# qwerty35/swarm_simulator

Hardware: AMD Instinct MI355X
Metric: agent-trajectories/sec (RBP plan: SFC+RSFC+QP) (higher is better)
Workload: dtype f64

## Files before the change

### swarm_simulator_amd/csrc/common/ipm_rows.h

```cpp
#pragma once
#include <cmath>
#include <cstddef>

#if defined(__HIPCC__)
#define IPM_ROW __host__ __device__ inline __attribute__((always_inline))
#define IPM_TABLE __constant__
#else
#define IPM_ROW inline
#define IPM_TABLE const
#endif
#if defined(__clang__)
#pragma clang fp contract(fast)
#endif

namespace ipm {

static IPM_TABLE double Qbase[36] = {720,  -1800, 1200,  0,     0,     -120, -1800, 4800,  -3600, 0,     600,   0,
                                     1200, -3600, 3600,  -1200, 0,     0,    0,     0,     -1200, 3600,  -3600, 1200,
                                     0,    600,   0,     -3600, 4800,  -1800, -120, 0,     0,     1200,  -1800, 720};
IPM_ROW size_t pair_index(int N, int qi, int qj) { return (size_t)qi * N - (size_t)qi * (qi + 1) / 2 + (qj - qi - 1); }

IPM_ROW double fast_rcp(double x) {
#if defined(__HIP_DEVICE_COMPILE__)
    double r = __builtin_amdgcn_rcp(x);
    r = fma(fma(-x, r, 1.0), r, r);
    r = fma(fma(-x, r, 1.0), r, r);
    return r;
#else
    return 1.0 / x;
#endif
}

IPM_ROW double weight(double s, double z, double dreg) { return z * fast_rcp(s + dreg * z); }

struct Build {
    double wgt, v, rg;
};
IPM_ROW Build build(double s, double z, double slack, double dreg) {
    Build b;
    b.rg = s - slack;
    b.wgt = weight(s, z, dreg);
    b.v = -b.wgt * (b.rg - s);
    return b;
}

IPM_ROW double step_limit(double s, double z, double ds, double dz) { return fmax(-ds * fast_rcp(s), -dz * fast_rcp(z)); }

struct Affine {
    double dza, dsa, cc, v, wz, lim;
};
IPM_ROW Affine affine(double s, double z, double slack, double ga, double dreg) {
    Affine a;
    const double rg = s - slack;
    const double iz = fast_rcp(z);
    const double wgt = weight(s, z, dreg);
    a.dza = wgt * (ga + rg - s);
    a.dsa = -s - s * a.dza * iz;
    a.cc = a.dsa * a.dza;
    a.lim = step_limit(s, z, a.dsa, a.dza);
    a.v = -wgt * (rg - s - a.cc * iz);
    a.wz = wgt * iz;
    return a;
}

struct Dir {
    double dz, ds;
};
IPM_ROW Dir direction(double s, double z, double slack_old, double ga, double gd, double dreg, double sigma_mu, double tt) {
    Dir d;
    const double rg = s - slack_old;
    const double iz = fast_rcp(z);
    const double w0 = weight(s, z, dreg);
    const double dza = w0 * (ga + rg - s);
    const double cc = (-s - s * dza * iz) * dza;
    const double rcc = s * z + cc - sigma_mu - tt;
    d.dz = w0 * (gd + rg - rcc * iz);
    d.ds = -(rcc + s * d.dz) * iz;
    return d;
}

struct State {
    double s, z, sz;
};
IPM_ROW State step_state(double s, double z, Dir d, double alpha) {
    State n;
    n.s = s + alpha * d.ds, n.z = z + alpha * d.dz;
    n.sz = n.s * n.z;
    return n;
}

struct Gondzio {
    double t, v;
};
IPM_ROW Gondzio gondzio(double s, double z, Dir d, double dreg, double atr, double mut) {
    Gondzio g;
    const double pr = (s + atr * d.ds) * (z + atr * d.dz);
    const double lo = 0.1 * mut, hi = 10.0 * mut;
    g.t = (pr < lo ? lo : (pr > hi ? hi : pr)) - pr;
    g.t = fmax(g.t, -hi);
    g.v = -weight(s, z, dreg) * g.t * fast_rcp(z);
    return g;
}

IPM_ROW double kmul(double s, double z, double dreg, double gd) { return weight(s, z, dreg) * gd; }

IPM_ROW double cand_strength(double s, double z) { return (z > s || s < 1e-6) ? fmax(z / s, 1e-300) : 0.0; }
constexpr double VERIFY_TOL = -1e-11;

IPM_ROW void acc_build(double (&S)[6], double (&yv)[3], double (&gz)[3], double wgt, double v, double zo, double sg, double n0, double n1,
                       double n2) {
    S[0] += wgt * n0 * n0, S[1] += wgt * n0 * n1, S[2] += wgt * n0 * n2;
    S[3] += wgt * n1 * n1, S[4] += wgt * n1 * n2, S[5] += wgt * n2 * n2;
    const double zz = sg * zo, vv = sg * v;
    gz[0] += zz * n0, gz[1] += zz * n1, gz[2] += zz * n2;
    yv[0] += vv * n0, yv[1] += vv * n1, yv[2] += vv * n2;
}
IPM_ROW void acc_aff(double (&S)[6], double v, double wz, double sg, double n0, double n1, double n2) {
    const double vv = sg * v, ww = sg * wz;
    S[0] += vv * n0, S[1] += vv * n1, S[2] += vv * n2;
    S[3] += ww * n0, S[4] += ww * n1, S[5] += ww * n2;
}
IPM_ROW void acc_kmul(double (&S)[6], double v, double sg, double n0, double n1, double n2) {
    const double vv = sg * v;
    S[0] += vv * n0, S[1] += vv * n1, S[2] += vv * n2;
}

IPM_ROW double pair_sign(bool a_lo) { return a_lo ? 1.0 : -1.0; }
IPM_ROW double pair_slack(bool a_lo, double n0, double n1, double n2, double xa0, double xa1, double xa2, double xb0, double xb1, double xb2,
                          double rsum) {
    const double e0 = a_lo ? xb0 - xa0 : xa0 - xb0, e1 = a_lo ? xb1 - xa1 : xa1 - xb1, e2 = a_lo ? xb2 - xa2 : xa2 - xb2;
    return n0 * e0 + n1 * e1 + n2 * e2 - rsum;
}
IPM_ROW double pair_dot(bool a_lo, double n0, double n1, double n2, double d0, double d1, double d2, double f0, double f1, double f2) {
    return a_lo ? n0 * (d0 - f0) + n1 * (d1 - f1) + n2 * (d2 - f2) : n0 * (f0 - d0) + n1 * (f1 - d1) + n2 * (f2 - d2);
}

IPM_ROW bool k0_factor_step(double* f, double (&Bp)[9], bool first) {
    bool ok = true;
    double A[9], Ej[9];
    for (int e = 0; e < 9; ++e) A[e] = f[e], Ej[e] = f[9 + e];
    if (!first)
        for (int r = 0; r < 3; ++r)
            for (int c = 0; c < 3; ++c) A[3 * r + c] -= Bp[3 * r] * Bp[3 * c] + Bp[3 * r + 1] * Bp[3 * c + 1] + Bp[3 * r + 2] * Bp[3 * c + 2];
    if (!(A[0] > 0)) ok = false;
    const double l00 = sqrt(A[0]), l10 = A[3] / l00, l20 = A[6] / l00;
    const double d11 = A[4] - l10 * l10;
    if (!(d11 > 0)) ok = false;
    const double l11 = sqrt(d11), l21 = (A[7] - l20 * l10) / l11;
    const double d22 = A[8] - l20 * l20 - l21 * l21;
    if (!(d22 > 0)) ok = false;
    const double l22 = sqrt(d22);
    f[0] = 1.0 / l00, f[1] = 0, f[2] = 0, f[3] = l10, f[4] = 1.0 / l11, f[5] = 0, f[6] = l20, f[7] = l21, f[8] = 1.0 / l22;
    for (int r = 0; r < 3; ++r) {
        const double o0 = Ej[r], o1 = Ej[3 + r], o2 = Ej[6 + r];
        const double x0 = o0 / l00, x1 = (o1 - x0 * l10) / l11, x2 = (o2 - x0 * l20 - x1 * l21) / l22;
        f[9 + 3 * r] = Bp[3 * r] = x0, f[10 + 3 * r] = Bp[3 * r + 1] = x1, f[11 + 3 * r] = Bp[3 * r + 2] = x2;
    }
    return ok;
}
template <class F>
IPM_ROW void k0_forward_step(F f, bool link, double (&y)[3], const double (&p)[3]) {
    if (link) {
        const F Bm = f - 9;
        y[0] -= Bm[0] * p[0] + Bm[1] * p[1] + Bm[2] * p[2];
        y[1] -= Bm[3] * p[0] + Bm[4] * p[1] + Bm[5] * p[2];
        y[2] -= Bm[6] * p[0] + Bm[7] * p[1] + Bm[8] * p[2];
    }
    y[0] = y[0] * f[0];
    y[1] = (y[1] - f[3] * y[0]) * f[4];
    y[2] = (y[2] - f[6] * y[0] - f[7] * y[1]) * f[8];
}
template <class F>
IPM_ROW void k0_backward_step(F f, bool link, double (&y)[3], const double (&p)[3]) {
    if (link) {
        const F Bm = f + 9;
        y[0] -= Bm[0] * p[0] + Bm[3] * p[1] + Bm[6] * p[2];
        y[1] -= Bm[1] * p[0] + Bm[4] * p[1] + Bm[7] * p[2];
        y[2] -= Bm[2] * p[0] + Bm[5] * p[1] + Bm[8] * p[2];
    }
    y[2] = y[2] * f[8];
    y[1] = (y[1] - f[7] * y[2]) * f[4];
    y[0] = (y[0] - f[3] * y[1] - f[6] * y[2]) * f[0];
}

}
```

### swarm_simulator_amd/csrc/kernels/qp.hip

```cpp
#include <algorithm>
#include <type_traits>
#include <vector>

#include "rbp_dev.h"

#pragma clang fp contract(fast)

#include "knot_lds.inc"
#include "common/ipm_rows.h"

#ifndef QP_THREADS
#define QP_THREADS 512
#endif
#define QP_MAX_ITERS 80
#ifndef QP_WARM_TAU
#define QP_WARM_TAU 1e-3
#endif
#ifndef QP_MU0
#define QP_MU0 3e-1
#endif
#ifndef QP_ROW_UNROLL
#define QP_ROW_UNROLL 2
#endif
#ifndef QP_ROW_PF
#define QP_ROW_PF 0
#endif
#ifndef QP_ROW_BLK
#define QP_ROW_BLK (QP_THREADS >= 512 ? 0 : 4)
#endif
#define QG(p) ((__attribute__((address_space(1))) double*)(p))
#define QGC(p) ((__attribute__((address_space(1))) const double*)(p))
#define QGF(p) ((__attribute__((address_space(1))) const float*)(p))
#ifndef QP_FAR_SLACK
#define QP_FAR_SLACK 0.7
#endif
#ifndef QP_SIGMA_POW
#define QP_SIGMA_POW 3
#endif
#ifndef QP_NBHD_GAMMA
#define QP_NBHD_GAMMA 1e-3
#endif
#ifndef QP_NBHD_BACKOFF
#define QP_NBHD_BACKOFF 0.8
#endif
#ifndef QP_STEP_FRAC
#define QP_STEP_FRAC 0.997
#endif
#ifndef QP_SFLOOR
#define QP_SFLOOR 1e-1
#endif
#ifndef QP_WAVES_PER_EU
#define QP_WAVES_PER_EU 2
#endif
#ifndef QP_CHAIN_PRIO
#define QP_CHAIN_PRIO 3
#endif
#ifndef QP_STAGE_BUFS
#define QP_STAGE_BUFS (QP_THREADS >= 512 ? 3 : 2)
#endif
#ifndef QP_STAGE_REGS
#define QP_STAGE_REGS (QP_THREADS >= 512 ? 0 : 2)
#endif
#ifndef QP_MID_FOLLOW
#define QP_MID_FOLLOW (QP_THREADS >= 512)
#endif
#ifndef QP_EARLY_TRIES
#define QP_EARLY_TRIES 2
#endif
#ifndef QP_EARLY_TOL
#define QP_EARLY_TOL 1e-6
#endif
#include "lh_layout.h"
#define PL_NC 256
#define PL_PMAX 160
#define PL_PBIG 192
__host__ __device__ inline int polish_pmax(int nk) { return nk <= 36 ? 112 : PL_PMAX; }
__host__ __device__ inline size_t polish_ws_doubles(int nj, int nk) {
    return PL_NC * 14 + (size_t)(PL_NC + 1) * nj * nk + PL_NC * PL_NC + 8 + lhp_size(PL_PBIG);
}
__host__ __device__ inline int polish_lds_doubles(int nk) {
    const int pm = polish_pmax(nk);
    return lhp_size(pm) + 3 * PL_NC + 3 * pm + (pm + 2 * PL_NC + 8) / 2 + 8;
}

namespace {
using namespace ipm;

#ifdef QP_PROFILE
#define PROF_DECL long long prof_t0 = wall_clock64(), prof_acc[12] = {0, 0, 0, 0, 0, 0, 0, 0, 0, 0, 0, 0}
#define PROF(i)                                \
    do {                                       \
        __syncthreads();                       \
        long long t_ = wall_clock64();         \
        prof_acc[i] += t_ - prof_t0;           \
        prof_t0 = t_;                          \
    } while (0)
#define PROF_FLUSH(scal)                                                         \
    do {                                                                         \
        if (threadIdx.x == 0)                                                    \
            for (int i_ = 0; i_ < 12; ++i_) scal[SC_PROF0 + i_] += (double)prof_acc[i_]; \
    } while (0)
#else
#define PROF_DECL
#define PROF(i)
#define PROF_FLUSH(scal)
#endif

struct QpDims {
    int N, M, oq;
    int nb, NF, npb;
    int nk, nj, ld;
    int ldb;
    int first;
    int ncol0;
    int ntile;
    size_t nslot_max;
};

__host__ __device__ inline QpDims make_dims(int N, int M, int first, int nb) {
    QpDims d;
    d.N = N, d.M = M, d.oq = 6 * M, d.nb = nb, d.NF = N - nb, d.npb = nb * (nb - 1) / 2;
    d.nk = 9 * nb, d.nj = M - 1, d.ld = d.nk + 1, d.first = first;
    d.ldb = d.nk <= 36 ? d.nk : ((d.nk + 15) & ~15);
    d.ncol0 = 6 + nb - 1, d.ntile = (nb * d.oq + 63) / 64;
    d.nslot_max = (size_t)d.ntile * 64 * (d.ncol0 + d.NF);
    return d;
}

struct QpWs {
    double *s, *z, *s2, *z2;
    double *rh;
    double *cc, *ds;
    double *cpacc;
    double *pwgt;
    double *dx, *dxa, *cvec;
    double *rbase, *rhs;
    double *Td, *To;
    double *Lf;
    double *boxlo, *boxhi;
    double *Lk, *Dk, *Ek;
    double *segsc;
    int *flist, *fcnt, *fbase;
    int *fnear;
    int *fperm, *frank;
    int *tile_base;
    int *wi_of;
    float* nrm;
    double* polish;
    double* prof;
};

__host__ __device__ inline size_t ws_int_count(int N, int M, int nbmax) {
    QpDims d = make_dims(N, M, 0, nbmax);
    return (size_t)nbmax * M * N  + 5 * (size_t)nbmax * M  + d.ntile + 1 + (size_t)nbmax * d.oq  +
           3 * (size_t)nbmax * M * N  + 8;
}

__host__ __device__ inline size_t ws_doubles(int N, int M, int nbmax) {
    QpDims d = make_dims(N, M, 0, nbmax);
    size_t n = 7 * d.nslot_max + 12 * (size_t)nbmax * d.oq + (size_t)(d.npb ? d.npb : 1) * d.oq + 3 * (size_t)nbmax * 3 * d.oq +
               2 * (size_t)d.nj * d.nk + (size_t)d.nj * d.ldb * d.ldb + 2 * (size_t)d.nj * (d.nk < 36 ? d.nk : 36) * (d.nk < 36 ? d.nk : 36) +
               (size_t)(d.nj > 1 ? d.nj - 1 : 1) * d.ldb * d.ldb + 4 +
               2 * (size_t)nbmax * M * 3 + 3 * (size_t)(M + 1) * 9 + M + 64 + (ws_int_count(N, M, nbmax) + 1) / 2 + 2 +
                polish_ws_doubles(d.nj, d.nk);
    return n;
}

__device__ inline QpWs carve(double* base, const QpDims& d, int nbmax) {
    QpDims dm = make_dims(d.N, d.M, 0, nbmax);
    QpWs w;
    double* p = base;
    w.s = p, p += dm.nslot_max;
    w.z = p, p += dm.nslot_max;
    w.s2 = p, p += dm.nslot_max;
    w.z2 = p, p += dm.nslot_max;
    w.rh = p, p += dm.nslot_max;
    w.cc = p, p += dm.nslot_max;
    w.ds = p, p += dm.nslot_max;
    w.cpacc = p, p += 12 * (size_t)nbmax * d.oq;
    w.pwgt = p, p += (size_t)(dm.npb ? dm.npb : 1) * d.oq;
    w.dx = p, p += (size_t)nbmax * 3 * d.oq;
    w.dxa = p, p += (size_t)nbmax * 3 * d.oq;
    w.cvec = p, p += (size_t)nbmax * 3 * d.oq;
    w.rbase = p, p += (size_t)dm.nj * dm.nk;
    w.rhs = p, p += (size_t)dm.nj * dm.nk;
    p += (4 - ((p - base) & 3)) & 3;
    w.Td = p, p += (size_t)dm.nj * dm.ldb * dm.ldb;
    w.To = p, p += (size_t)(dm.nj > 1 ? dm.nj - 1 : 1) * dm.ldb * dm.ldb;
    w.Lf = p, p += 2 * (size_t)dm.nj * (dm.nk < 36 ? dm.nk : 36) * (dm.nk < 36 ? dm.nk : 36);
    w.boxlo = p, p += (size_t)nbmax * d.M * 3;
    w.boxhi = p, p += (size_t)nbmax * d.M * 3;
    w.Lk = p, p += (size_t)(d.M + 1) * 9;
    w.Dk = p, p += (size_t)(d.M + 1) * 9;
    w.Ek = p, p += (size_t)(d.M + 1) * 9;
    w.segsc = p, p += d.M;
    int* ip = (int*)p;
    w.flist = ip, ip += (size_t)nbmax * d.M * d.N;
    w.fnear = ip, ip += (size_t)nbmax * d.M;
    w.fcnt = ip, ip += (size_t)nbmax * d.M;
    w.fbase = ip, ip += (size_t)nbmax * d.M;
    w.fperm = ip, ip += (size_t)nbmax * d.M;
    w.frank = ip, ip += (size_t)nbmax * d.M;
    w.tile_base = ip, ip += dm.ntile + 1;
    w.wi_of = ip, ip += (size_t)nbmax * d.oq;
    w.nrm = (float*)ip;
    w.polish = p + (ws_int_count(d.N, d.M, nbmax) + 1) / 2 + 2;
    w.prof = nullptr;
    return w;
}

template <int CTRL>
__device__ __forceinline__ double dpp_f64(double v) {
    const int lo = __builtin_amdgcn_update_dpp(0, __double2loint(v), CTRL, 0xf, 0xf, false);
    const int hi = __builtin_amdgcn_update_dpp(0, __double2hiint(v), CTRL, 0xf, 0xf, false);
    return __hiloint2double(hi, lo);
}
__device__ __forceinline__ double red_op(double a, double b, int op) { return op == 0 ? a + b : (op == 1 ? fmax(a, b) : fmin(a, b)); }
__device__ __forceinline__ double rl(double v, int lane) {
    return __hiloint2double(__builtin_amdgcn_readlane(__double2hiint(v), lane), __builtin_amdgcn_readlane(__double2loint(v), lane));
}
__device__ __forceinline__ double wave_red(double v, int op ) {
    v = red_op(v, dpp_f64<0xB1>(v), op);
    v = red_op(v, dpp_f64<0x4E>(v), op);
    v = red_op(v, dpp_f64<0x141>(v), op);
    v = red_op(v, dpp_f64<0x140>(v), op);
    return red_op(red_op(rl(v, 0), rl(v, 16), op), red_op(rl(v, 32), rl(v, 48), op), op);
}
__device__ inline double block_reduce(double v, int op , double* red) {
    v = wave_red(v, op);
    const int wave = threadIdx.x >> 6, lane = threadIdx.x & 63;
    if (lane == 0) red[wave] = v;
    __syncthreads();
    double r = red[0];
    for (int i = 1; i < QP_THREADS / 64; ++i) r = red_op(r, red[i], op);
    __syncthreads();
    return r;
}

__device__ void mission_constants(const QpDims& d, const double* T, QpWs& w) {
    const int M = d.M;
    for (int m = threadIdx.x; m < M; m += QP_THREADS) w.segsc[m] = pow(T[m + 1] - T[m], -5.0);
    for (int j = threadIdx.x; j <= M; j += QP_THREADS) {
        double* L = w.Lk + 9 * j;
        for (int e = 0; e < 9; ++e) L[e] = 0;
        if (j >= 1 && j < M) {
            const double r = (T[j] - T[j - 1]) / (T[j + 1] - T[j]);
            L[0] = (1 + r) * (1 + r), L[1] = -2 * r * (1 + r), L[2] = r * r;
            L[3] = 1 + r, L[4] = -r, L[5] = 0;
            L[6] = 1, L[7] = 0, L[8] = 0;
        }
    }
    __syncthreads();
    for (int j = threadIdx.x; j <= M; j += QP_THREADS) {
        double* D = w.Dk + 9 * j;
        double* E = w.Ek + 9 * j;
        for (int e = 0; e < 9; ++e) D[e] = 0, E[e] = 0;
        if (j >= 1 && j < M) {
            const double sl = pow(T[j] - T[j - 1], -5.0), sr = pow(T[j + 1] - T[j], -5.0);
            const double* L = w.Lk + 9 * j;
            double QL[9];
            for (int a = 0; a < 3; ++a)
                for (int b = 0; b < 3; ++b) {
                    double s = 0;
                    for (int c = 0; c < 3; ++c) s += Qbase[6 * (3 + a) + 3 + c] * sl * L[3 * c + b];
                    QL[3 * a + b] = s;
                }
            for (int a = 0; a < 3; ++a)
                for (int b = 0; b < 3; ++b) {
                    double s = 0;
                    for (int c = 0; c < 3; ++c) s += L[3 * c + a] * QL[3 * c + b];
                    D[3 * a + b] = 2 * (s + Qbase[6 * a + b] * sr);
                }
            if (j + 1 < M) {
                const double* Ln = w.Lk + 9 * (j + 1);
                for (int a = 0; a < 3; ++a)
                    for (int b = 0; b < 3; ++b) {
                        double s = 0;
                        for (int c = 0; c < 3; ++c) s += Qbase[6 * a + 3 + c] * sr * Ln[3 * c + b];
                        E[3 * a + b] = 2 * s;
                    }
            }
        }
    }
    __syncthreads();
}

enum { PASS_INIT = 0, PASS_BUILD, PASS_AFF, PASS_STEP, PASS_PRESOLVE, PASS_CAND, PASS_VERIFY, PASS_CAND_GEO,
       PASS_UPBUILD  };

constexpr bool pass_in_blocks(int pass) {
    return pass == PASS_BUILD || pass == PASS_AFF || pass == PASS_STEP || pass == PASS_UPBUILD || pass == PASS_CAND || pass == PASS_VERIFY ||
           pass == PASS_CAND_GEO;
}

struct PassIO {
    double mu0, s_floor, dreg, sigma_mu, alpha;
    double sum0, sum1, sum2, vmax, vmin;
};

#define QP_POLISH_PART 1
#include "qp_polish.inc"
#undef QP_POLISH_PART

#define QP_META_G 160
struct SweepMeta {
    unsigned short fbase[QP_META_G];
    unsigned char grp[QP_META_G], near[QP_META_G], all[QP_META_G];
    int tile_base[16];
};
struct RowCtx {
    const SweepMeta* meta;
    const PolishWs* pw;
    double* scal;
    int mission;
    int lds_avail;
    QpDims d;
    QpWs w;
    const double* ctrl;
    const float* normals;
    const double* radius;
};

__device__ __forceinline__ double fast_rsqrt(double x) {
    double y = __builtin_amdgcn_rsq(x);
    const double h = 0.5 * x;
    y = fma(y, fma(-h * y, y, 0.5), y);
    y = fma(y, fma(-h * y, y, 0.5), y);
    return y;
}

template <int PASS, bool PRE = false>
__device__ __forceinline__ void row_op(double slack, double ga, double gd, size_t r, const QpWs& w, PassIO& io, double cw, double& wgt,
                                       double& v, double& zo, double s_in = 0.0, double z_in = 0.0) {
    constexpr bool rd_sz = PASS == PASS_BUILD || PASS == PASS_AFF || PASS == PASS_STEP || PASS == PASS_UPBUILD || PASS == PASS_CAND;
    double s = 0.0, z = 0.0;
    if (rd_sz) s = PRE ? s_in : QGC(w.s)[r], z = PRE ? z_in : QGC(w.z)[r];
    if (PASS == PASS_INIT) {
        const double s0 = slack < io.s_floor ? io.s_floor : slack;
        w.s[r] = s0;
        w.z[r] = io.mu0 / s0;
    } else if (PASS == PASS_BUILD) {
        const Build b = build(s, z, slack, io.dreg);
        wgt = b.wgt, v = b.v, zo = z;
        io.sum0 += cw * s * z;
        io.vmax = fmax(io.vmax, fabs(b.rg));
    } else if (PASS == PASS_AFF) {
        const Affine a = affine(s, z, slack, ga, io.dreg);
        io.vmax = fmax(io.vmax, a.lim);
        io.sum0 += cw * s * z, io.sum1 += cw * (s * a.dza + z * a.dsa), io.sum2 += cw * a.cc;
        v = a.v, wgt = a.wz;
    } else if (PASS == PASS_STEP) {
        const Dir d = direction(s, z, slack, ga, gd, io.dreg, io.sigma_mu, 0.0);
        io.vmax = fmax(io.vmax, step_limit(s, z, d.ds, d.dz));
    } else if (PASS == PASS_UPBUILD) {
        const State n = step_state(s, z, direction(s, z, slack + io.alpha * gd, ga, gd, io.dreg, io.sigma_mu, 0.0), io.alpha);
        QG(w.s2)[r] = n.s, QG(w.z2)[r] = n.z;
        io.vmin = fmin(io.vmin, n.sz);
        const Build b = build(n.s, n.z, slack, io.dreg);
        wgt = b.wgt, v = b.v, zo = n.z;
        io.sum0 += cw * n.s * n.z;
        io.vmax = fmax(io.vmax, fabs(b.rg));
    } else if (PASS == PASS_PRESOLVE) {
        io.vmax = fmax(io.vmax, -slack);
    } else if (PASS == PASS_CAND) {
        wgt = cand_strength(s, z);
        QG(w.cc)[r] = wgt;
        v = slack;
    } else if (PASS == PASS_CAND_GEO) {
        wgt = slack < QP_WARM_TAU ? (slack < 1e-8 ? 1e3 : 1.0) : 0.0;
        QG(w.cc)[r] = wgt;
        v = slack;
    } else if (PASS == PASS_VERIFY) {
        const double sn = slack - gd;
        QG(w.ds)[r] = sn;
        io.vmax = fmax(io.vmax, -sn);
        if (sn < VERIFY_TOL && QGC(w.cc)[r] == 0.0) {
            QG(w.cc)[r] = 1.0;
            wgt = 1.0;
        }
    }
}
// ... 1514 lines not shown
            double* A = w.Td + (size_t)j * ld * ld;
            const double* B = j > 0 ? w.To + (size_t)(j - 1) * ld * ld : nullptr;
            double* C = j + 1 < d.nj ? w.To + (size_t)j * ld * ld : nullptr;
            if (!factor_knot_tiled<false>(A, B, C, ld, NT, flag)) return false;
        }
    }
    __threadfence_block();
    __syncthreads();
    return true;
}

template <bool LDS>
__device__ __forceinline__ void trisolve_fwd(const double* L, int ld, int n, double* v, int lane) {
    const int NT = n / 16, i = lane & 15;
    for (int p = 0; p < NT; ++p) {
        double a[16];
        const double* dp = L + (size_t)(16 * p + i) * ld + 16 * p;
        const d4 v0 = ld4T<LDS>(dp), v1 = ld4T<LDS>(dp + 4), v2 = ld4T<LDS>(dp + 8), v3 = ld4T<LDS>(dp + 12);
#pragma unroll
        for (int k = 0; k < 4; ++k) a[k] = v0[k], a[4 + k] = v1[k], a[8 + k] = v2[k], a[12 + k] = v3[k];
        double x = v[16 * p + i], dgl = 1.0;
#pragma unroll
        for (int k = 0; k < 16; ++k) dgl = (i == k) ? a[k] : dgl;
        const double inv = 1.0 / dgl;
#pragma unroll
        for (int c = 0; c < 16; ++c) {
            const double xc = rl(x, c) * rl(inv, c);
            x = (i == c) ? xc : (i > c ? x - a[c] * xc : x);
        }
        if (lane < 16) v[16 * p + i] = x;
        for (int r0 = 16 * (p + 1); r0 < n; r0 += 64) {
            const int r = r0 + lane;
            const bool act = r < n;
            const double* rp = L + (size_t)(act ? r : 0) * ld + 16 * p;
            const d4 u0 = ld4T<LDS>(rp), u1 = ld4T<LDS>(rp + 4), u2 = ld4T<LDS>(rp + 8), u3 = ld4T<LDS>(rp + 12);
            double sv = 0;
#pragma unroll
            for (int k = 0; k < 4; ++k)
                sv += u0[k] * rl(x, k) + u1[k] * rl(x, 4 + k) + u2[k] * rl(x, 8 + k) + u3[k] * rl(x, 12 + k);
            if (act) v[r] -= sv;
        }
        __builtin_amdgcn_fence(__ATOMIC_SEQ_CST, "wavefront");
        __builtin_amdgcn_wave_barrier();
    }
}

template <bool LDS>
__device__ __forceinline__ void trisolve_bwd(const double* L, int ld, int n, double* v, int lane) {
    const int NT = n / 16, i = lane & 15;
    for (int p = NT - 1; p >= 0; --p) {
        double at[16];
#pragma unroll
        for (int k = 0; k < 16; ++k) at[k] = ldT<LDS>(L + (size_t)(16 * p + k) * ld + 16 * p + i);
        double x = v[16 * p + i], dgl = 1.0;
#pragma unroll
        for (int k = 0; k < 16; ++k) dgl = (i == k) ? at[k] : dgl;
        const double inv = 1.0 / dgl;
#pragma unroll
        for (int c = 15; c >= 0; --c) {
            const double xc = rl(x, c) * rl(inv, c);
            x = (i == c) ? xc : (i < c ? x - at[c] * xc : x);
        }
        if (lane < 16) v[16 * p + i] = x;
        for (int k0 = 0; k0 < 16 * p; k0 += 64) {
            const int k = k0 + lane;
            const bool act = k < 16 * p;
            const double* cp = L + (size_t)(16 * p) * ld + (act ? k : 0);
            double sv = 0;
#pragma unroll
            for (int c = 0; c < 16; ++c) sv += ldT<LDS>(cp + (size_t)c * ld) * rl(x, c);
            if (act) v[k] -= sv;
        }
        __builtin_amdgcn_fence(__ATOMIC_SEQ_CST, "wavefront");
        __builtin_amdgcn_wave_barrier();
    }
}

__device__ void solve_tiled(const QpDims& d, const QpWs& w, double* rhs, double* lds, int lds_avail) {
    const int nk = d.nk, ld = d.ldb, tid = threadIdx.x, wave = tid >> 6, lane = tid & 63;
    double* cur = lds;
    double* oth = lds + ld;
    double* part = lds + 2 * ld;
    const int ldl = ld + 2;
    double* Lst = part + QP_THREADS;
    const bool staged = 2 * ld + QP_THREADS + ld * ldl <= lds_avail;
    for (int j = 0; j < d.nj; ++j) {
        for (int r = tid; r < ld; r += QP_THREADS) cur[r] = r < nk ? rhs[(size_t)j * nk + r] : 0.0;
        __syncthreads();
        if (j > 0) {
            const double* Lo = w.To + (size_t)(j - 1) * ld * ld;
            const int i = tid & 15;
            for (int r0 = 0; r0 < nk; r0 += QP_THREADS / 16) {
                const int r = r0 + (tid >> 4);
                double sv = 0;
                if (r < nk)
                    for (int c = i; c < ld; c += 16) sv += Lo[(size_t)r * ld + c] * oth[c];
                sv += __shfl_xor(sv, 8), sv += __shfl_xor(sv, 4), sv += __shfl_xor(sv, 2), sv += __shfl_xor(sv, 1);
                if (r < nk && i == 0) cur[r] -= sv;
            }
            __syncthreads();
        }
        if (staged) {
            stage_block(Lst, ldl, w.Td + (size_t)j * ld * ld, ld);
            __syncthreads();
        }
        if (wave == 0) {
            if (staged)
                trisolve_fwd<true>(Lst, ldl, ld, cur, lane);
            else
                trisolve_fwd<false>(w.Td + (size_t)j * ld * ld, ld, ld, cur, lane);
        }
        __syncthreads();
        for (int r = tid; r < nk; r += QP_THREADS) rhs[(size_t)j * nk + r] = cur[r];
        double* t = cur;
        cur = oth, oth = t;
    }
    __threadfence_block();
    for (int j = d.nj - 1; j >= 0; --j) {
        __syncthreads();
        for (int r = tid; r < ld; r += QP_THREADS) cur[r] = r < nk ? rhs[(size_t)j * nk + r] : 0.0;
        __syncthreads();
        if (j + 1 < d.nj) {
            const double* Lo = w.To + (size_t)j * ld * ld;
            if (ld <= QP_THREADS) {
                const int ng = QP_THREADS / ld, c = tid % ld, g = tid / ld;
                if (g < ng) {
                    double sv = 0;
                    for (int r = g; r < ld; r += ng) sv += Lo[(size_t)r * ld + c] * oth[r];
                    part[tid] = sv;
                }
                __syncthreads();
                if (tid < nk) {
                    double sv = 0;
                    for (int q = 0; q < ng; ++q) sv += part[q * ld + tid];
                    cur[tid] -= sv;
                }
            } else {
                for (int c = tid; c < nk; c += QP_THREADS) {
                    double sv = 0;
                    for (int r = 0; r < ld; ++r) sv += Lo[(size_t)r * ld + c] * oth[r];
                    cur[c] -= sv;
                }
            }
            __syncthreads();
        }
        if (staged) {
            stage_block(Lst, ldl, w.Td + (size_t)j * ld * ld, ld);
            __syncthreads();
        }
        if (wave == 0) {
            if (staged)
                trisolve_bwd<true>(Lst, ldl, ld, cur, lane);
            else
                trisolve_bwd<false>(w.Td + (size_t)j * ld * ld, ld, ld, cur, lane);
        }
        __syncthreads();
        for (int r = tid; r < nk; r += QP_THREADS) rhs[(size_t)j * nk + r] = cur[r];
        double* t = cur;
        cur = oth, oth = t;
    }
    __threadfence_block();
    __syncthreads();
}

__device__ void init_block_pads(const QpDims& d, const QpWs& w) {
    const int nk = d.nk, ld = d.ldb;
    if (ld == nk) return;
    const int npad = ld - nk;
    for (int it = threadIdx.x; it < d.nj * npad * ld; it += QP_THREADS) {
        const int j = it / (npad * ld), q = it % (npad * ld), r = nk + q / ld, c = q % ld;
        double* A = w.Td + (size_t)j * ld * ld;
        A[(size_t)r * ld + c] = r == c ? 1.0 : 0.0;
        A[(size_t)c * ld + r] = r == c ? 1.0 : 0.0;
    }
}

template <int ROLE>
__device__ __forceinline__ bool factor_dispatch(const QpDims& d, const QpWs& w, double* lA, int* flag, int lds_avail, const AsmArgs* asmb) {
    if (d.nk <= 36) {
        switch (d.nk) {
            case 9: return twisted_factor<9, ROLE>(d, w, flag, lA, asmb);
            case 18: return twisted_factor<18, ROLE>(d, w, flag, lA, asmb);
            case 27: return twisted_factor<27, ROLE>(d, w, flag, lA, asmb);
            default: return twisted_factor<36, ROLE>(d, w, flag, lA, asmb);
        }
    }
    if (ROLE != 0) return true;
    return factor_tiled(d, w, flag, lA, lds_avail);
}

template <int ROLE>
__device__ __forceinline__ void solve_dispatch(const QpDims& d, const QpWs& w, double* rhs, double* lA, int lds_avail, SolveOut so = SolveOut{nullptr, nullptr, 0}) {
    if (d.nk <= 36) {
        switch (d.nk) {
            case 9: solve_staged<9, ROLE>(d, w, rhs, lA, so); break;
            case 18: solve_staged<18, ROLE>(d, w, rhs, lA, so); break;
            case 27: solve_staged<27, ROLE>(d, w, rhs, lA, so); break;
            default: solve_staged<36, ROLE>(d, w, rhs, lA, so); break;
        }
        return;
    }
    if (ROLE != 1) solve_tiled(d, w, rhs, lA, lds_avail);
}


struct BlkArgs {
    int nk, nj, ldb, lds_avail;
    double *Td, *To, *Lf;
    double* Ek;
    double* prof;
};
__device__ __forceinline__ int uni(int v) { return __builtin_amdgcn_readfirstlane(v); }
template <class T>
__device__ __forceinline__ T* uni(T* p) {
    const unsigned long long v = (unsigned long long)p;
    const unsigned lo = __builtin_amdgcn_readfirstlane((unsigned)v), hi = __builtin_amdgcn_readfirstlane((unsigned)(v >> 32));
    return (T*)(((unsigned long long)hi << 32) | lo);
}
__device__ __forceinline__ void blk_unpack(const BlkArgs& b, QpDims& d, QpWs& w) {
    d = QpDims{};
    w = QpWs{};
    d.nk = uni(b.nk), d.nj = uni(b.nj), d.ldb = uni(b.ldb), d.ld = d.nk + 1;
    w.Td = uni(b.Td), w.To = uni(b.To), w.Lf = uni(b.Lf), w.Ek = uni(b.Ek), w.prof = uni(b.prof);
}
__device__ __forceinline__ AsmArgs uni(const AsmArgs& A) {
    return AsmArgs{uni(A.cpacc), uni(A.pwgt), uni(A.Lk), uni(A.Dk), uni(A.normals), uni(A.Td), uni(A.N), uni(A.M), uni(A.nb), uni(A.first), uni(A.oq), uni(A.ldb)};
}
__device__ __noinline__ bool factor_entry_chain(BlkArgs b, AsmArgs A, double* lds, int* flag) {
    QpDims d;
    QpWs w;
    blk_unpack(b, d, w);
    const AsmArgs Au = uni(A);
    return factor_dispatch<0>(d, w, uni(lds), uni(flag), uni(b.lds_avail), &Au);
}
__device__ __noinline__ bool factor_entry_assemble(BlkArgs b, AsmArgs A, double* lds, int* flag) {
    QpDims d;
    QpWs w;
    blk_unpack(b, d, w);
    const AsmArgs Au = uni(A);
    return factor_dispatch<1>(d, w, uni(lds), uni(flag), uni(b.lds_avail), &Au);
}
__device__ __noinline__ bool factor_entry_follow(BlkArgs b, AsmArgs A, double* lds, int* flag) {
    QpDims d;
    QpWs w;
    blk_unpack(b, d, w);
    const AsmArgs Au = uni(A);
    return factor_dispatch<2>(d, w, uni(lds), uni(flag), uni(b.lds_avail), &Au);
}
__device__ __forceinline__ bool factor_entry(const BlkArgs& b, const AsmArgs& A, double* lds, int* flag) {
    const int wave = threadIdx.x >> 6;
    if (b.nk <= 36 && wave >= 4) return factor_entry_assemble(b, A, lds, flag);
    if (b.nk <= 36 && wave >= 2) return factor_entry_follow(b, A, lds, flag);
    return factor_entry_chain(b, A, lds, flag);
}
__device__ __noinline__ void solve_entry_chain(BlkArgs b, double* rhs, double* lds, SolveOut so) {
    QpDims d;
    QpWs w;
    blk_unpack(b, d, w);
    solve_dispatch<0>(d, w, uni(rhs), uni(lds), uni(b.lds_avail), SolveOut{uni(so.dx_out), uni(so.Lk), uni(so.oq), uni(so.rhs_mode), uni(so.cpacc), uni(so.rbase), so.sigma_mu});
}
__device__ __noinline__ void solve_entry_stage(BlkArgs b, double* rhs, double* lds, SolveOut so) {
    QpDims d;
    QpWs w;
    blk_unpack(b, d, w);
    solve_dispatch<1>(d, w, uni(rhs), uni(lds), uni(b.lds_avail), SolveOut{uni(so.dx_out), uni(so.Lk), uni(so.oq), uni(so.rhs_mode), uni(so.cpacc), uni(so.rbase), so.sigma_mu});
}
__device__ __forceinline__ void solve_entry(const BlkArgs& b, double* rhs, double* lds, SolveOut so = SolveOut{nullptr, nullptr, 0}) {
    if (b.nk <= 36 && (threadIdx.x >> 6) >= 2)
        solve_entry_stage(b, rhs, lds, so);
    else
        solve_entry_chain(b, rhs, lds, so);
}

#define QP_POLISH_PART 2
#include "qp_polish.inc"
#undef QP_POLISH_PART

#ifdef QP_TRACE
#ifndef QP_TRACE_BATCH
#define QP_TRACE_BATCH 0
#endif
#define TRC(slot, expr)                                                         \
    do {                                                                        \
        if (batch == QP_TRACE_BATCH && pass_index == 0 && iter < 100) {                       \
            const double v_ = (expr);                                           \
            if (tid == 0) trc[iter * 16 + (slot)] = v_;                         \
        }                                                                       \
    } while (0)
__device__ double trc_sum(const double* p, size_t n, double* red) {
    double a = 0;
    for (size_t i = threadIdx.x; i < n; i += QP_THREADS) a += fabs(p[i]);
    return block_reduce(a, 0, red);
}
#else
#define TRC(slot, expr)
#endif

__device__ __forceinline__ bool qp_setup_batch(const DevSession& S, RowCtx& c, double* ctrl, const double* T, int mission, int first, int nb,
                                               int* flag, double* lds, int& frozen_free_rows, double far_R, int& nfar) {
    const int tid = threadIdx.x, N = S.N;
    const QpDims& d = c.d;
    const QpWs& w = c.w;
    const int M = d.M;
    mission_constants(d, T, const_cast<QpWs&>(w));
    init_block_pads(d, w);

    {
        const int need = nb * S.max_boxes + (M + 2) + (nb * M + 1) / 2 + 1;
        const bool stage = need <= c.lds_avail;
        double* bt_l = lds;
        double* T_l = lds + nb * S.max_boxes;
        int* sel_l = stage ? (int*)(T_l + M + 2) : w.fcnt;
        if (stage) {
            for (int it = tid; it < nb * S.max_boxes; it += QP_THREADS)
                bt_l[it] = S.sfc_time[((size_t)mission * N + first + it / S.max_boxes) * S.max_boxes + it % S.max_boxes];
            for (int it = tid; it <= M; it += QP_THREADS) T_l[it] = T[it];
            __syncthreads();
        }
        for (int a = tid; a < nb; a += QP_THREADS) {
            const int qa = first + a;
            int nbx = S.sfc_count[(size_t)mission * N + qa];
            if (nbx <= 0) {
                atomicCAS(&S.status[mission], 0, (int)RBP_ERR_BAD_ARGUMENT);
                nbx = 1;
            }
            const double* bt = stage ? bt_l + a * S.max_boxes : S.sfc_time + ((size_t)mission * N + qa) * S.max_boxes;
            const double* Tt = stage ? T_l : T;
            int bi = 0;
            for (int m = 0; m < M; ++m) {
                while (bi < nbx && bt[bi] < Tt[m + 1]) bi++;
                sel_l[a * M + m] = bi < nbx ? bi : nbx - 1;
            }
        }
        __threadfence_block();
        __syncthreads();
        for (int it = tid; it < nb * M * 3; it += QP_THREADS) {
            const int am = it / 3, k = it % 3, a = am / M;
            const double* bx = S.sfc_box + ((size_t)mission * N + first + a) * S.max_boxes * 6 + 6 * sel_l[am];
            w.boxlo[(size_t)am * 3 + k] = bx[k];
            w.boxhi[(size_t)am * 3 + k] = bx[3 + k];
        }
        __threadfence_block();
        __syncthreads();
    }
    for (int it = tid; it < nb * 3; it += QP_THREADS) {
        const int a = it / 3, k = it % 3, qa = first + a;
        const double* st = S.start + ((size_t)mission * N + qa) * 9;
        const double* gl = S.goal + ((size_t)mission * N + qa) * 9;
        const double h0 = T[1] - T[0], hT = T[M] - T[M - 1];
        double* x = ctrl + ((size_t)qa * 3 + k) * d.oq;
        x[0] = st[k], x[1] = x[0] + h0 * st[k + 3] / 5, x[2] = 2 * x[1] - x[0] + h0 * h0 * st[k + 6] / 20;
        double* xe = x + 6 * (M - 1);
        xe[5] = gl[k], xe[4] = xe[5] - hT * gl[k + 3] / 5, xe[3] = 2 * xe[4] - xe[5] + hT * hT * gl[k + 6] / 20;
    }
    __threadfence();
    __syncthreads();
    if (__hip_atomic_load(&S.status[mission], __ATOMIC_RELAXED, __HIP_MEMORY_SCOPE_AGENT) != 0) return false;

    for (int it = tid; it < nb * M; it += QP_THREADS) {
        const int a = it / M, seg = it % M, qa = first + a;
        const double ra = c.radius[qa];
        const double* lo = w.boxlo + ((size_t)a * M + seg) * 3;
        const double* hi = w.boxhi + ((size_t)a * M + seg) * 3;
        int cnt = 0, nfar_g = 0;
        int* fl = w.flist + (size_t)it * N;
        double xa6[6][3];
#pragma unroll
        for (int i = 0; i < 6; ++i)
#pragma unroll
            for (int e = 0; e < 3; ++e) xa6[i][e] = ctrl[((size_t)qa * 3 + e) * d.oq + 6 * seg + i];
        for (int f0 = 0; f0 < N && N > 1; f0 += 4) {
            bool keep4[4], far4[4];
            float nvq[4][3];
            double cf[4][6][3];
#pragma unroll
            for (int q = 0; q < 4; ++q) {
                const int f = f0 + q < N ? f0 + q : N - 1;
                const bool a_first = qa < f;
                const int lo_ = a_first ? qa : f, hi_ = a_first ? f : qa;
                const float* nv = c.normals + (pair_index(N, lo_ == hi_ ? 0 : lo_, lo_ == hi_ ? 1 : hi_) * M + seg) * 3;
#pragma unroll
                for (int e = 0; e < 3; ++e) nvq[q][e] = nv[e];
#pragma unroll
                for (int i = 0; i < 6; ++i)
#pragma unroll
                    for (int e = 0; e < 3; ++e) cf[q][i][e] = ctrl[((size_t)f * 3 + e) * d.oq + 6 * seg + i];
            }
#pragma unroll
            for (int q = 0; q < 4; ++q) {
                const int f = f0 + q;
                const bool a_first = qa < f;
                const double sg = a_first ? 1.0 : -1.0;
                const double n0 = sg * (double)nvq[q][0], n1 = sg * (double)nvq[q][1], n2 = sg * (double)nvq[q][2];
                const double mx = fmax(n0 * lo[0], n0 * hi[0]) + fmax(n1 * lo[1], n1 * hi[1]) + fmax(n2 * lo[2], n2 * hi[2]);
                const double rr = ra + c.radius[f < N ? f : 0];
                bool keep = false;
                double smin = 1e300;
#pragma unroll
                for (int i = 0; i < 6; ++i) {
                    const double nd = n0 * cf[q][i][0] + n1 * cf[q][i][1] + n2 * cf[q][i][2];
                    if (!(nd - rr - mx > 1e-6)) keep = true;
                    smin = fmin(smin, nd - rr - (n0 * xa6[i][0] + n1 * xa6[i][1] + n2 * xa6[i][2]));
                }
                keep4[q] = keep && f < N && !(f >= first && f < first + nb);
                far4[q] = smin > far_R;
            }
#pragma unroll
            for (int q = 0; q < 4; ++q)
                if (keep4[q]) {
                    if (far4[q])
                        fl[N - 1 - nfar_g++] = f0 + q;
                    else
                        fl[cnt++] = f0 + q;
                }
        }
        w.fnear[it] = cnt;
        w.fcnt[it] = cnt + nfar_g;
    }
    __threadfence_block();
    __syncthreads();
    if (tid == 0) flag[0] = 0, flag[1] = 0;
    __syncthreads();
    for (int it = tid; it < nb * M; it += QP_THREADS) {
        int acc = 0;
        for (int o = 0; o < it; ++o) acc += w.fcnt[o];
        w.fbase[it] = acc;
        const int seg = it % M;
        atomicAdd(flag, w.fnear[it] * ((seg == 0 || seg == M - 1) ? (M == 1 ? 0 : 3) : 6));
        atomicAdd(flag + 1, w.fcnt[it] - w.fnear[it]);
    }
    __threadfence_block();
    __syncthreads();
    frozen_free_rows = *flag;
    nfar = flag[1];
    __syncthreads();
    for (int it = tid; it < nb * M; it += QP_THREADS) {
        const int ci = w.fcnt[it];
        int rank = 0;
        for (int o = 0; o < nb * M; ++o) {
            const int co = w.fcnt[o];
            rank += (co > ci || (co == ci && o < it)) ? 1 : 0;
        }
        w.fperm[rank] = it;
        w.frank[it] = rank;
    }
    __threadfence_block();
    __syncthreads();
    for (int t = tid; t <= d.ntile; t += QP_THREADS) {
        int base = 0;
        for (int o = 0; o < t; ++o) base += 64 * (d.ncol0 + w.fcnt[w.fperm[(64 * o) / 6]]);
        w.tile_base[t] = base;
    }
    for (int wi = tid; wi < nb * d.oq; wi += QP_THREADS) {
        const int grp = w.fperm[wi / 6], a = grp / M, seg = grp - a * M;
        w.wi_of[a * d.oq + 6 * seg + wi % 6] = wi;
    }
    __threadfence_block();
    __syncthreads();
    for (int it = tid; it < nb * M * 6; it += QP_THREADS) {
        const int as = it / 6, i = it % 6, a = as / M, seg = as % M, qa = first + a, j6 = 6 * seg + i;
        const int cnt = w.fcnt[as], cn = w.fnear[as];
        const int* fl = w.flist + (size_t)as * N;
        const int wi = 6 * w.frank[as] + i;
        const size_t r0 = (size_t)w.tile_base[wi >> 6] + (wi & 63) + (size_t)d.ncol0 * 64;
        float* nr = w.nrm + (size_t)w.fbase[as] * 3;
        const double ra = c.radius[qa];
        for (int i0 = 0; i0 < cnt; i0 += 4) {
            int fq[4];
            float nvq[4][3];
            double cfq[4][3];
#pragma unroll
            for (int q = 0; q < 4; ++q) {
                const int e = i0 + q < cnt ? i0 + q : cnt - 1;
                fq[q] = fl[e < cn ? e : N - 1 - (e - cn)];
            }
#pragma unroll
            for (int q = 0; q < 4; ++q) {
                const int f = fq[q];
                const bool a_first = qa < f;
                const float* nv = c.normals + (pair_index(N, a_first ? qa : f, a_first ? f : qa) * M + seg) * 3;
#pragma unroll
                for (int e = 0; e < 3; ++e) nvq[q][e] = nv[e], cfq[q][e] = ctrl[((size_t)f * 3 + e) * d.oq + j6];
            }
#pragma unroll
            for (int q = 0; q < 4; ++q) {
                const int idx = i0 + q, f = fq[q];
                if (idx < cnt) {
                    const float sgf = qa < f ? 1.0f : -1.0f;
                    const double n0 = (double)(sgf * nvq[q][0]), n1 = (double)(sgf * nvq[q][1]), n2 = (double)(sgf * nvq[q][2]);
                    if (i == 0) nr[3 * idx] = sgf * nvq[q][0], nr[3 * idx + 1] = sgf * nvq[q][1], nr[3 * idx + 2] = sgf * nvq[q][2];
                    w.rh[r0 + (size_t)idx * 64] = n0 * cfq[q][0] + n1 * cfq[q][1] + n2 * cfq[q][2] - (ra + c.radius[f]);
                }
            }
        }
    }
    __threadfence_block();
    __syncthreads();
    return true;
}

__device__ __forceinline__ int qp_batch_body(const DevSession& S, double* ws_base, size_t ws_stride, int mission, int batch, int nbmax,
                                             int reset_cost, int lds_doubles, int pass_index, double far_R) {
    const int tid = threadIdx.x;
    if (S.status[mission] != 0) return 0;
    const int N = S.N, M = __builtin_amdgcn_readfirstlane(S.Mk[mission]), MS = S.M;
    const int first = batch * nbmax;
    const int nb = min(nbmax, N - first);
    if (nb <= 0) return 0;
    RowCtx c;
    c.meta = nullptr;
    c.scal = S.scalars + (size_t)mission * SC_N, c.mission = mission, c.lds_avail = lds_doubles - 32;
    c.d = make_dims(N, M, first, nb);
    c.w = carve(ws_base + (size_t)mission * ws_stride, c.d, nbmax);
    double* ctrl = S.ctrl + (size_t)mission * N * 3 * 6 * MS;
    c.ctrl = ctrl;
    c.normals = S.rsfc_normal + (size_t)mission * S.npair * MS * 3;
    c.radius = S.radius + (size_t)mission * N;
    const QpDims& d = c.d;
    const QpWs& w = c.w;
    const double* T = S.T + (size_t)mission * (MS + 1);
    double* scal = S.scalars + (size_t)mission * SC_N;

    extern __shared__ __attribute__((aligned(16))) double lds_raw[];
    double* red = lds_raw;
    int* flag = (int*)(lds_raw + 16);
    double* lds = lds_raw + 32;
    double* lA = lds;
#ifdef QP_PROFILE
    const BlkArgs ba{d.nk, d.nj, d.ldb, c.lds_avail, w.Td, w.To, w.Lf, w.Ek, scal};
#else
    const BlkArgs ba{d.nk, d.nj, d.ldb, c.lds_avail, w.Td, w.To, w.Lf, w.Ek, nullptr};
#endif
    double* red2 = red;
    int* flag2 = flag;

    PROF_DECL;
    int frozen_free_rows = 0, nfar = 0;
    if (!qp_setup_batch(S, c, ctrl, T, mission, first, nb, flag, lds, frozen_free_rows, far_R, nfar)) return 0;
    PROF(8);
    PassIO io;
    __shared__ RowCtx c_lds;
#if QP_ROW_BLK > 0
    __shared__ SweepMeta meta_lds;
    const bool meta_ok = nb * d.M <= QP_META_G && d.ntile + 1 <= 16 && d.N <= 256 && (size_t)nb * d.M * d.N < 65536;
    __syncthreads();
    if (meta_ok) {
        for (int rk = tid; rk < nb * d.M; rk += QP_THREADS) {
            const int g = w.fperm[rk];
            meta_lds.grp[rk] = (unsigned char)g, meta_lds.near[rk] = (unsigned char)w.fnear[g], meta_lds.all[rk] = (unsigned char)w.fcnt[g];
            meta_lds.fbase[rk] = (unsigned short)w.fbase[g];
        }
        for (int t = tid; t <= d.ntile; t += QP_THREADS) meta_lds.tile_base[t] = w.tile_base[t];
    }
    c.meta = meta_ok ? &meta_lds : nullptr;
#endif
    __syncthreads();
    if (tid == 0) c_lds = c;
    __syncthreads();
    io.mu0 = QP_MU0, io.s_floor = QP_SFLOOR, io.dreg = 1e-9, io.sigma_mu = 0, io.alpha = 0;
    io.vmax = 0;
    row_pass<PASS_PRESOLVE>(c, io);
    const double pin_viol = block_reduce(io.vmax, 1, red);
    if (pin_viol > 1e-6) {
        if (tid == 0) {
            atomicCAS(&S.status[mission], 0, (int)RBP_ERR_QP_FAILED);
#ifndef QP_PROFILE
            scal[SC_PROF0 + 1] = 1000.0 * batch + 1, scal[SC_PROF0 + 2] = pin_viol;
#endif
        }
        return 0;
    }
    const double nrows_free = (double)((size_t)(d.oq - 6) * (6 * d.nb + d.npb)) + (double)frozen_free_rows;
    bool ok = false;
    int it_count = 0, polished = 0, early_tries = 0, fail_reason = 3;
    double gap_next = 0, pres_next = 0, kkt_ipm = 0;
    double flops = 0, rows_swept = 0, row_bytes = 0, sweep_bytes = 0;
    const double blk_doubles = d.nk <= 36 ? 5.0 * (d.nk * (d.nk + 1) / 2) + 5.0 * d.nk : 8.0 * d.ldb * d.ldb;
    const double bytes_sweeps = 88.0 * frozen_free_rows + 64.0 * (double)(d.oq - 6) * (6.0 * d.nb + 2.0 * d.npb) + 288.0 * (double)d.nb * (d.oq - 6);
    const double bytes_iter = bytes_sweeps + 8.0 * (double)d.nj * blk_doubles;
    PolishWs pw;
    pw.cand = (Cand*)w.polish;
    pw.V = w.polish + PL_NC * 14;
    pw.Sg = pw.V + (size_t)(PL_NC + 1) * d.nj * d.nk;
    pw.ncand = (int*)(pw.Sg + PL_NC * PL_NC);
    pw.Lbig = pw.Sg + PL_NC * PL_NC + 8;
    row_pass<PASS_INIT>(c, io);
    __threadfence_block();
    __syncthreads();
#ifdef QP_TRACE
    double* trc = S.coef + (size_t)mission * N * 3 * 6 * MS;
#endif
    for (int iter = 0; iter < QP_MAX_ITERS; ++iter) {
        it_count = iter;
        PROF(0);
        if (iter == 0) {
            io.sum0 = 0, io.vmax = 0;
            SWEEP(PASS_BUILD);
        }
        PROF(1);
        const double gap = iter == 0 ? block_reduce(io.sum0, 0, red) : gap_next;
        const double pres = iter == 0 ? block_reduce(io.vmax, 1, red) : pres_next;
        __threadfence_block();
        __syncthreads();
        double dmax, gmax;
        rbase_from_acc(c, dmax, gmax);
        const double dres = block_reduce(dmax, 1, red) / (1.0 + block_reduce(gmax, 1, red));
        const double mu = gap / nrows_free;
        rows_swept += nrows_free;
        kkt_ipm = fmax(pres, fmax(dres, mu));
        TRC(0, gap); TRC(1, pres); TRC(2, dres); TRC(3, trc_sum(w.rbase, (size_t)d.nj * d.nk, red)); TRC(4, trc_sum(w.cpacc, (size_t)12 * d.nb * d.oq, red));
        if (pres < 1e-9 && dres < 1e-9 && mu < 1e-10) {
            ok = true;
            break;
        }
        if (pres < 1e-6 && dres < 1e-9 && mu < 1e-13) {
            ok = true;
            break;
        }
        if (pres < 1e-9 && dres < 1e-7 && mu < 1e-14) {
            ok = true;
            break;
        }
        PROF(2);
        const bool polish_first = pass_index > 0 && iter == 0;
        const bool early = early_tries < QP_EARLY_TRIES && pres < QP_EARLY_TOL && dres < QP_EARLY_TOL &&
                           mu < (early_tries == 0 ? QP_EARLY_TOL : 1e-2 * QP_EARLY_TOL);
        if (S.p.polish && (polish_first || early)) {
            if (!polish_first) early_tries++;
            const int acc = polish_entry(c, pw, lds, red2, flag2, polish_first ? 1 : 0);
            __syncthreads();
            PROF(0);
#ifdef QP_POLSTATS
            if (tid == 0 && !polish_first) scal[25] += (early_tries == 1), scal[26] += (early_tries == 1 && acc == 0), scal[27] += (early_tries == 2), scal[29] += (early_tries == 2 && acc == 0);
#endif
            if (acc == 0) {
                ok = true, polished = 1;
                break;
            }
        }
        if (d.nk > 36)
            assemble_blocks(c, lds);
        else if (ASM_HELPERS == 0 && !QP_FOLLOW_ASM)
            assemble_blocks_lds(asm_args(c), d.nj, lds);
        PROF(3);
        __threadfence_block();
        __syncthreads();
        TRC(5, trc_sum(w.Td, (size_t)d.nj * d.ldb * d.ldb, red));
        if (!factor_entry(ba, asm_args(c), lA, flag)) {
            fail_reason = 2;
            break;
        }
        flops += d.nk <= 36 ? (double)d.nj * ((7.0 / 6.0) * d.nk * (double)d.nk * d.nk + 6.0 * d.nk * (double)d.nk)
                            : (double)d.nj * (7.0 / 3.0) * d.nk * (double)d.nk * d.nk;
        PROF(4);
        TRC(6, trc_sum(d.nk <= 36 ? w.Lf : w.Td, d.nk <= 36 ? (size_t)d.nj * 2 * d.nk * d.nk : (size_t)d.nj * d.ldb * d.ldb, red));
#ifndef QP_TRACE
        if (d.nk <= 36) {
            PROF(5);
            solve_entry(ba, w.rhs, lA, SolveOut{w.dxa, w.Lk, d.oq, 1, w.cpacc, w.rbase, 0.0});
            PROF(6);
        } else
#endif
        {
            rhs_from_acc(c, false, 0.0);
            __threadfence_block();
            __syncthreads();
            PROF(5);
            TRC(7, trc_sum(w.rhs, (size_t)d.nj * d.nk, red));
            solve_entry(ba, w.rhs, lA);
            PROF(6);
            TRC(8, trc_sum(w.rhs, (size_t)d.nj * d.nk, red));
            apply_F(d, w, w.rhs, w.dxa);
            __threadfence_block();
            __syncthreads();
        }
        io.sum0 = io.sum1 = io.sum2 = 0, io.vmax = 1.0;
        PROF(5);
        SWEEP(PASS_AFF);
        PROF(7);
        const double a_aff = 1.0 / block_reduce(io.vmax, 1, red);
        const double q0 = block_reduce(io.sum0, 0, red), q1 = block_reduce(io.sum1, 0, red), q2 = block_reduce(io.sum2, 0, red);
        const double mu_aff = (q0 + a_aff * q1 + a_aff * a_aff * q2) / nrows_free;
        TRC(9, a_aff); TRC(10, mu_aff);
        double sigma = mu_aff / mu;
        sigma = QP_SIGMA_POW == 2 ? sigma * sigma : (QP_SIGMA_POW == 4 ? sigma * sigma * sigma * sigma : sigma * sigma * sigma);
        io.sigma_mu = sigma * mu;
        __threadfence_block();
        __syncthreads();
        PROF(8);
#ifndef QP_TRACE
        if (d.nk <= 36) {
            PROF(5);
            solve_entry(ba, w.rhs, lA, SolveOut{w.dx, w.Lk, d.oq, 2, w.cpacc, w.rbase, io.sigma_mu});
            PROF(6);
        } else
#endif
        {
            rhs_from_acc(c, true, io.sigma_mu);
            __threadfence_block();
            __syncthreads();
            PROF(5);
            TRC(11, trc_sum(w.rhs, (size_t)d.nj * d.nk, red));
            solve_entry(ba, w.rhs, lA);
            PROF(6);
            TRC(12, trc_sum(w.rhs, (size_t)d.nj * d.nk, red));
            apply_F(d, w, w.rhs, w.dx);
            __threadfence_block();
            __syncthreads();
        }
        flops += 2.0 * d.nj * 4.0 * d.nk * (double)d.nk;
        io.vmax = QP_STEP_FRAC;
        PROF(5);
        SWEEP(PASS_STEP);
        PROF(9);
        double alpha = QP_STEP_FRAC / block_reduce(io.vmax, 1, red);
        TRC(13, alpha);
        __threadfence_block();
        __syncthreads();
        double applied = 0;
        for (int bt = 0; bt < 40; ++bt) {
            const double delta = alpha - applied;
            {
                double* xb = ctrl + (size_t)first * 3 * d.oq;
                const int nx = d.nb * 3 * d.oq;
                for (int i0 = tid; i0 < nx; i0 += 4 * QP_THREADS) {
                    double xv[4], dv4[4];
#pragma unroll
                    for (int q = 0; q < 4; ++q) {
                        const int i = i0 + q * QP_THREADS;
                        xv[q] = i < nx ? xb[i] : 0.0, dv4[q] = i < nx ? w.dx[i] : 0.0;
                    }
#pragma unroll
                    for (int q = 0; q < 4; ++q) {
                        const int i = i0 + q * QP_THREADS;
                        if (i < nx) xb[i] = xv[q] + delta * dv4[q];
                    }
                }
            }
            __threadfence_block();
            __syncthreads();
            io.alpha = alpha, io.sum0 = 0, io.vmax = 0, io.vmin = 1e300;
            SWEEP(PASS_UPBUILD);
            applied = alpha;
            gap_next = block_reduce(io.sum0, 0, red);
            pres_next = block_reduce(io.vmax, 1, red);
            const double pmin = block_reduce(io.vmin, 2, red);
            rows_swept += nrows_free;
            __threadfence_block();
            __syncthreads();
            if (pmin >= QP_NBHD_GAMMA * gap_next / nrows_free) break;
            alpha *= QP_NBHD_BACKOFF;
        }
        {
            double* t0 = c.w.s;
            c.w.s = c.w.s2, c.w.s2 = t0;
            t0 = c.w.z, c.w.z = c.w.z2, c.w.z2 = t0;
            if (tid == 0) c_lds.w.s = c.w.s, c_lds.w.s2 = c.w.s2, c_lds.w.z = c.w.z, c_lds.w.z2 = c.w.z2;
            __syncthreads();
        }
        rows_swept += 2 * nrows_free;
        row_bytes += bytes_iter, sweep_bytes += bytes_sweeps;
        PROF(10);
        PROF(11);
    }
    if (!ok && nfar > 0) {
        if (tid == 0) scal[SC_IPM_ITERS] += it_count, scal[SC_FLOPS] += flops, scal[SC_ROWS] += rows_swept;
        return 1;
    }
    if (!ok) {
        if (tid == 0) {
            atomicCAS(&S.status[mission], 0, (int)RBP_ERR_QP_FAILED);
#ifndef QP_PROFILE
            scal[SC_PROF0 + 1] = 1000.0 * batch + fail_reason, scal[SC_PROF0 + 2] = it_count;
#endif
        }
        return 0;
    }
    if (S.p.polish && !polished) {
        int acc = polish_entry(c, pw, lds, red2, flag2, 0);
        if (acc == 3) {
            __syncthreads();
            acc = polish_entry(c, pw, lds, red2, flag2, 2);
        }
        polished = acc == 0 ? 1 : 0;
#ifdef QP_POLSTATS
        if (tid == 0) scal[30] += 1, scal[31] += polished;
#endif
        PROF(0);
#ifndef QP_PROFILE
        if (acc != 0 && tid == 0) scal[SC_PROF0] += 1000.0 * batch + acc;
#endif
        __syncthreads();
    }
    __syncthreads();
    if (S.p.polish && !polished && nfar > 0) {
        if (tid == 0) scal[SC_IPM_ITERS] += it_count, scal[SC_FLOPS] += flops, scal[SC_ROWS] += rows_swept;
        return 1;
    }
    const double kkt = polished ? red[12] : kkt_ipm;
    double obj = 0;
    for (int it = tid; it < d.nb * 3 * M; it += QP_THREADS) {
        const int a = it / (3 * M), k = (it / M) % 3, m = it % M;
        const double sc = w.segsc[m];
        const double* xs = ctrl + ((size_t)(first + a) * 3 + k) * d.oq + 6 * m;
        double q = 0;
        for (int i = 0; i < 6; ++i)
            for (int jj = 0; jj < 6; ++jj) q += Qbase[6 * i + jj] * xs[i] * xs[jj];
        obj += q * sc;
    }
    obj = block_reduce(obj, 0, red);
    if (tid == 0) {
        if (reset_cost) scal[SC_TOTAL_COST] = 0;
        scal[SC_TOTAL_COST] += obj;
        scal[SC_IPM_ITERS] += it_count;
        scal[SC_QP_SOLVED] += 1;
        scal[SC_POLISHED] += polished;
        scal[SC_KKT_MAX] = fmax(scal[SC_KKT_MAX], kkt);
        scal[SC_FLOPS] += flops;
        scal[SC_ROWS] += rows_swept;
#ifndef QP_LHSTATS
        scal[SC_ROW_BYTES] += row_bytes;
        scal[SC_SWEEP_BYTES] += sweep_bytes;
#endif
    }
    PROF_FLUSH(scal);
    return 0;
}

__device__ void restore_dummy(const DevSession& s, int mission, int first, int nbmax) {
    const int N = s.N, MS = s.M, PS = MS + 1, M = s.Mk[mission], P = M + 1, oq = 6 * M;
    const int nb = min(nbmax, N - first);
    double* ctrl = s.ctrl + (size_t)mission * N * 3 * 6 * MS;
    for (int it = threadIdx.x; it < nb * 3 * oq; it += QP_THREADS) {
        const int j6 = it % oq, k = (it / oq) % 3, qi = first + it / (3 * oq);
        const int m = j6 / 6, j = j6 % 6;
        const float* tr = s.init_traj + (size_t)mission * N * PS * 3 + (size_t)qi * P * 3;
        ctrl[((size_t)qi * 3 + k) * oq + j6] = dummy_ctrl_point(tr, m, j, k);
    }
}

__device__ __noinline__ int qp_batch_body_outofline(const DevSession* Sg, double* ws_base, size_t ws_stride, int mission, int batch, int nbmax,
                                                    int reset_cost, int lds_doubles, int pass_index, double far_R) {
    const DevSession S = *Sg;
    return qp_batch_body(S, uni(ws_base), ws_stride, uni(mission), uni(batch), uni(nbmax), uni(reset_cost), uni(lds_doubles), uni(pass_index), far_R);
}
__device__ __noinline__ void qp_finish_schedule(const DevSession* Sg, double* ws_base, size_t ws_stride, int mission, int passes, int biter, int nbmax,
                                               int lds_doubles, int it0, int l0) {
    const DevSession S = *Sg;
    ws_base = uni(ws_base), mission = uni(mission), passes = uni(passes), biter = uni(biter), nbmax = uni(nbmax), lds_doubles = uni(lds_doubles);
    it0 = uni(it0), l0 = uni(l0);
    for (int it = it0; it < passes; ++it)
        for (int l = (it == it0 ? l0 : 0); l < biter; ++l) {
            const bool failed = it == it0 && l == l0;
            for (int attempt = failed ? 1 : 0; attempt < 2; ++attempt) {
                if (attempt == 1) {
#ifndef QP_PROFILE
                    if (threadIdx.x == 0) S.scalars[(size_t)mission * SC_N + SC_PROF0 + 3] += 1;
#endif
                    restore_dummy(S, mission, l * nbmax, nbmax);
                    __threadfence_block();
                    __syncthreads();
                }
                const double far_R = (attempt == 0 && it == 0 && S.p.polish && S.p.far_slack > 0.0) ? S.p.far_slack : 1e300;
                const int again = uni(qp_batch_body_outofline(Sg, ws_base, ws_stride, mission, l, nbmax, (int)(l == 0), lds_doubles, it, far_R));
                __threadfence_block();
                __syncthreads();
                if (!again) break;
            }
        }
}

__global__ __launch_bounds__(QP_THREADS, QP_WAVES_PER_EU) void qp_batch_kernel(DevSession S, double* ws_base, size_t ws_stride, int passes,
                                                               int biter, int nbmax, int lds_doubles) {
    const int mission = S.qp_order ? __builtin_amdgcn_readfirstlane(S.qp_order[blockIdx.x]) : (int)blockIdx.x;
    const long long t_start = wall_clock64();
    __shared__ DevSession S_lds;
    if (threadIdx.x == 0) S_lds = S;
    __syncthreads();
    int stop_it = -1, stop_l = 0;
    for (int it = 0; it < passes && stop_it < 0; ++it)
        for (int l = 0; l < biter; ++l) {
            const double far_R = (it == 0 && S.p.polish && S.p.far_slack > 0.0) ? S.p.far_slack : 1e300;
            const int again = qp_batch_body(S, ws_base, ws_stride, mission, l, nbmax, (int)(l == 0), lds_doubles, it, far_R);
            __threadfence_block();
            __syncthreads();
            if (again) {
                stop_it = it, stop_l = l;
                break;
            }
        }
    if (stop_it >= 0) qp_finish_schedule(&S_lds, ws_base, ws_stride, mission, passes, biter, nbmax, lds_doubles, stop_it, stop_l);
    if (S.qp_cost && threadIdx.x == 0) S.qp_cost[mission] = (unsigned long long)(wall_clock64() - t_start) + 1;
}

__global__ __launch_bounds__(256) void qp_order_kernel(DevSession S) {
    const int k = blockIdx.x * blockDim.x + threadIdx.x;
    if (k >= S.K) return;
    const unsigned long long c = S.qp_cost[k];
    int rank = 0;
    bool valid = c != 0;
    for (int o = 0; o < S.K; ++o) {
        const unsigned long long co = S.qp_cost[o];
        valid = valid && co != 0;
        rank += (co > c || (co == c && o < k)) ? 1 : 0;
    }
    if (valid)
        S.qp_order[rank] = k;
    else
        S.qp_order[k] = k;
}

}

#ifndef QP_SUFFIX
#define QP_SUFFIX _w2
#endif
#define QP_CAT2(a, b) a##b
#define QP_CAT(a, b) QP_CAT2(a, b)
size_t QP_CAT(planner_workspace_bytes, QP_SUFFIX)(int N, int M, int batch_size_eff) {
    return (ws_doubles(N, M, batch_size_eff) * sizeof(double) + 255) & ~size_t(255);
}

static size_t qp_lds_bytes(int bs, int M) {
    const int nk = 9 * bs;
    const int nkw = std::min(nk, 36);
    size_t lds = sizeof(double) * (2 * (size_t)((nk + 15) & ~15) + QP_THREADS + 32) + 16;
    lds = std::max(lds, sizeof(double) * (size_t)(std::max(polish_lds_doubles(nk), polish_lds_doubles(nkw)) + 18 * (M - 1) + 32) + 16);
    lds = std::max(lds, sizeof(double) * (16 + (size_t)QP_STAGE_BUFS * 2 * (nkw * KL_LD + KL_I) + (size_t)(M - 1) * nkw + 2 + 6 * KS_VLEN + 2 * 64 + 64));
    lds = std::max(lds, sizeof(double) * (size_t)(2 * kl_area_doubles(nkw) + 128 + (QP_FOLLOW_ASM ? 2 : ASM_HELPERS) * ASML_DOUBLES(nkw, nkw / 9) + 32) + 16);
    if (nk > 36 && nk <= 72) {
        const size_t lb = (size_t)((nk + 15) & ~15);
        lds = std::max(lds, sizeof(double) * (3 * lb * (lb + 2) + 34) + 16);
    }
    return lds;
}

void QP_CAT(launch_planner, QP_SUFFIX)(const DevSession& s, void* qp_ws, size_t ws_bytes_per_mission, hipStream_t st) {
    const int M = s.M;
    const BatchSchedule sched = batch_schedule(s.p.sequential, s.p.batch_size, s.p.batch_iter, s.N);
    const int bs = sched.bs, biter = sched.biter;
    launch_planner_prologue(s, st);
    if (biter > 0) {
        if (bs > QP_MAX_NB) {
            (void)rbp_set_error(RBP_ERR_BAD_ARGUMENT, "launch_planner: batch wider than the QP kernel supports");
            return;
        }
        const size_t lds = qp_lds_bytes(bs, M);
        (void)hipFuncSetAttribute((const void*)qp_batch_kernel, hipFuncAttributeMaxDynamicSharedMemorySize, (int)lds);
        if (s.p.iteration > 0 && s.qp_order) hipLaunchKernelGGL(qp_order_kernel, dim3((s.K + 255) / 256), dim3(256), 0, st, s);
        if (s.p.iteration > 0)
            hipLaunchKernelGGL(qp_batch_kernel, dim3(s.K), dim3(QP_THREADS), lds, st, s, (double*)qp_ws,
                               ws_bytes_per_mission / sizeof(double), s.p.iteration, biter, bs, (int)(lds / sizeof(double)) - 2);
    }
#ifdef QP_TRACE
    return;
#endif
    launch_planner_epilogue(s, st);
}
```

### swarm_simulator_amd/csrc/kernels/qp_polish.inc

```

#if QP_POLISH_PART == 1

struct Cand {
    double n[3], t[3];
    double slack, snap_val;
    double strength;
    int row, knot, a, b, snap_idx, pad;
};

struct PolishWs {
    Cand* cand;
    double* V;
    double* Sg;
    int* ncand;
    double* Lbig;
};

#define WSYNC()                                             \
    do {                                                    \
        __builtin_amdgcn_fence(__ATOMIC_SEQ_CST, "wavefront"); \
        __builtin_amdgcn_wave_barrier();                    \
    } while (0)

__device__ __forceinline__ int wave_min_int(int v) {
    v = min(v, __builtin_amdgcn_update_dpp(0, v, 0xB1, 0xf, 0xf, false));
    v = min(v, __builtin_amdgcn_update_dpp(0, v, 0x4E, 0xf, 0xf, false));
    v = min(v, __builtin_amdgcn_update_dpp(0, v, 0x141, 0xf, 0xf, false));
    v = min(v, __builtin_amdgcn_update_dpp(0, v, 0x140, 0xf, 0xf, false));
    return min(min(__builtin_amdgcn_readlane(v, 0), __builtin_amdgcn_readlane(v, 16)),
               min(__builtin_amdgcn_readlane(v, 32), __builtin_amdgcn_readlane(v, 48)));
}
__device__ __forceinline__ void wave_argmax(double& best, int& bidx) {
    const double top = wave_red(bidx >= 0 ? best : -1e300, 1);
    const int idx = wave_min_int(bidx >= 0 && best == top ? bidx : 0x7fffffff);
    best = top, bidx = idx == 0x7fffffff ? -1 : idx;
}

__device__ __forceinline__ void knot_of(const QpDims& d, const QpWs& w, int j6, int& knot, double t[3]) {
    const int m = j6 / 6, i = j6 % 6;
    if (i < 3) {
        knot = m;
        t[0] = t[1] = t[2] = 0;
        t[i] = 1;
    } else {
        knot = m + 1;
        const double* L = w.Lk + 9 * (m + 1) + 3 * (i - 3);
        t[0] = L[0], t[1] = L[1], t[2] = L[2];
    }
}

__device__ __forceinline__ void emit_cand(const QpDims& d, const QpWs& w, const PolishWs& pw, size_t r, int j6, int a, int b, double n0,
                                          double n1, double n2, double slack, int snap_idx, double snap_val, double strength) {
    const int idx = atomicAdd(pw.ncand, 1);
    if (idx >= PL_NC) return;
    Cand& c = pw.cand[idx];
    c.n[0] = n0, c.n[1] = n1, c.n[2] = n2;
    knot_of(d, w, j6, c.knot, c.t);
    c.slack = slack, c.snap_val = snap_val, c.strength = strength;
    c.row = (int)r, c.a = a, c.b = b, c.snap_idx = snap_idx, c.pad = 0;
}

#else
__device__ __forceinline__ int cand_meta(const Cand& c) {
    return c.a | ((c.b + 1) << 8) | ((c.n[0] != 0.0) << 16) | ((c.n[1] != 0.0) << 17) | ((c.n[2] != 0.0) << 18);
}
__device__ __forceinline__ bool meta_has(int meta, int agent, int k) {
    return meta < 0 || ((((meta >> 16) >> k) & 1) && (agent == (meta & 255) || agent == ((meta >> 8) & 255) - 1));
}
__device__ __forceinline__ double cand_dot(const Cand& c, const double* vec, int nk, int colmeta = -1) {
    const double* blk = vec + (size_t)(c.knot - 1) * nk;
    double s = 0;
#pragma unroll
    for (int k = 0; k < 3; ++k) {
        if (c.n[k] == 0.0) continue;
        double ta = 0;
        if (meta_has(colmeta, c.a, k)) {
            const double* pa = blk + (c.a * 3 + k) * 3;
            ta = c.t[0] * pa[0] + c.t[1] * pa[1] + c.t[2] * pa[2];
        }
        if (c.b >= 0 && meta_has(colmeta, c.b, k)) {
            const double* pb = blk + (c.b * 3 + k) * 3;
            ta -= c.t[0] * pb[0] + c.t[1] * pb[1] + c.t[2] * pb[2];
        }
        s += c.n[k] * ta;
    }
    return s;
}

__device__ void k0_factor3(const QpDims& d, const QpWs& w, double* f3, int* flag) {
    for (int it = threadIdx.x; it < 18 * d.nj; it += QP_THREADS) {
        const int jj = it / 18, e = it % 18, j = jj + 1;
        f3[it] = e < 9 ? w.Dk[9 * j + e] : (jj + 1 < d.nj ? w.Ek[9 * j + (e - 9)] : 0.0);
    }
    __syncthreads();
    if (threadIdx.x == 0) {
        int ok = 1;
        double Bp[9] = {0, 0, 0, 0, 0, 0, 0, 0, 0};
        for (int jj = 0; jj < d.nj; ++jj)
            if (!k0_factor_step(f3 + 18 * jj, Bp, jj == 0)) ok = 0;
        *flag = !ok;
    }
    __syncthreads();
}

constexpr int K0_BLK = 6;
__device__ __forceinline__ void k0_solve3(const double* f3g, int nj, int nk, double* col, int sub) {
    typedef __attribute__((address_space(1))) double gdb;
    const kl_lds* f3 = (const kl_lds*)f3g;
    gdb* y = QG(col) + sub * 3;
    constexpr int B = K0_BLK;
    double cur[B][3], nxt[B][3];
    double p[3] = {0, 0, 0};
#pragma unroll
    for (int u = 0; u < B; ++u) {
        const int jx = u < nj ? u : nj - 1;
#pragma unroll
        for (int e = 0; e < 3; ++e) cur[u][e] = y[(size_t)jx * nk + e];
    }
    for (int j0 = 0; j0 < nj; j0 += B) {
#pragma unroll
        for (int u = 0; u < B; ++u) {
            const int jx = j0 + B + u < nj ? j0 + B + u : nj - 1;
#pragma unroll
            for (int e = 0; e < 3; ++e) nxt[u][e] = y[(size_t)jx * nk + e];
        }
#pragma unroll
        for (int u = 0; u < B; ++u) {
            const int jj = j0 + u;
            if (jj < nj) {
                k0_forward_step(f3 + 18 * jj, jj > 0, cur[u], p);
                y[(size_t)jj * nk] = p[0] = cur[u][0], y[(size_t)jj * nk + 1] = p[1] = cur[u][1], y[(size_t)jj * nk + 2] = p[2] = cur[u][2];
            }
        }
#pragma unroll
        for (int u = 0; u < B; ++u)
#pragma unroll
            for (int e = 0; e < 3; ++e) cur[u][e] = nxt[u][e];
    }
#pragma unroll
    for (int u = 0; u < B; ++u) {
        const int jx = nj - 1 - u >= 0 ? nj - 1 - u : 0;
#pragma unroll
        for (int e = 0; e < 3; ++e) cur[u][e] = y[(size_t)jx * nk + e];
    }
    for (int jt = nj - 1; jt >= 0; jt -= B) {
#pragma unroll
        for (int u = 0; u < B; ++u) {
            const int jx = jt - B - u >= 0 ? jt - B - u : 0;
#pragma unroll
            for (int e = 0; e < 3; ++e) nxt[u][e] = y[(size_t)jx * nk + e];
        }
#pragma unroll
        for (int u = 0; u < B; ++u) {
            const int jj = jt - u;
            if (jj >= 0) {
                k0_backward_step(f3 + 18 * jj, jj + 1 < nj, cur[u], p);
                y[(size_t)jj * nk] = p[0] = cur[u][0], y[(size_t)jj * nk + 1] = p[1] = cur[u][1], y[(size_t)jj * nk + 2] = p[2] = cur[u][2];
            }
        }
#pragma unroll
        for (int u = 0; u < B; ++u)
#pragma unroll
            for (int e = 0; e < 3; ++e) cur[u][e] = nxt[u][e];
    }
}

__device__ __noinline__ void col_solve3_fn(int nj_v, int nk_v, int nb_v, double* V_v, const Cand* cand_v, const double* f3_v, int with_grad_v, int c0_v, int c1_v) {
    const int nj = __builtin_amdgcn_readfirstlane(nj_v), nk = __builtin_amdgcn_readfirstlane(nk_v), nb = __builtin_amdgcn_readfirstlane(nb_v);
    const int with_grad = __builtin_amdgcn_readfirstlane(with_grad_v), c0 = __builtin_amdgcn_readfirstlane(c0_v), c1 = __builtin_amdgcn_readfirstlane(c1_v);
    double* V = uni(V_v);
    const Cand* cand = uni(cand_v);
    const double* f3 = uni(f3_v);
    const int nred = nj * nk, ng = with_grad ? nb * 3 : 0;
    for (int it = threadIdx.x; it < ng + (c1 - c0) * 6; it += QP_THREADS) {
        if (it < ng) {
            k0_solve3(f3, nj, nk, V, it);
            continue;
        }
        const int ci = c0 + (it - ng) / 6, side = ((it - ng) % 6) / 3, k = (it - ng) % 3;
        const Cand& cd = cand[ci];
        const int ag = side == 0 ? cd.a : cd.b;
        if (ag < 0 || cd.n[k] == 0.0) continue;
        k0_solve3(f3, nj, nk, V + (size_t)(1 + ci) * nred, ag * 3 + k);
    }
}
__device__ __forceinline__ void col_solve3(const QpDims& d, const PolishWs& pw, const double* f3, bool with_grad, int c0, int c1) {
    col_solve3_fn(d.nj, d.nk, d.nb, pw.V, pw.cand, f3, with_grad ? 1 : 0, c0, c1);
    __threadfence_block();
    __syncthreads();
}

__device__ __forceinline__ double rl_dyn(double v, int lane) {
    const int lo = __builtin_amdgcn_readlane(__double2loint(v), lane);
    const int hi = __builtin_amdgcn_readlane(__double2hiint(v), lane);
    return __hiloint2double(hi, lo);
}

#include "lh_inverse.inc"

__device__ int lh_wave(int n, const double* Sg, int ldS, const double* dv, double* zc, double* tv, double* yv, double* wv, int* P, int* inP,
                       int* banned, double* Lc, int* shared_int, int pmax, double* str, bool big, double* stats = nullptr, int resume_nP = -1,
                       int n_prev = 0) {
    const int lane = threadIdx.x & 63;
    kl_lds* Wl = big ? nullptr : (kl_lds*)Lc;
    double* Wg = big ? Lc : nullptr;
    int* rem = (int*)tv;
    int nP = 0;
    double dmax = 0;
    const bool resume = resume_nP >= 0;
    for (int a = lane; a < n; a += 64) {
        if (!resume || a >= n_prev)
            zc[a] = 0;
        else
            zc[a] = fmax(zc[a], 0.0);
        inP[a] = 0, banned[a] = 0;
        dmax = fmax(dmax, fabs(dv[a]));
    }
    dmax = wave_red(dmax, 1);
    const double wtol = 1e-12 * fmax(1.0, dmax);
    if (resume) {
        nP = resume_nP;
        WSYNC();
        for (int b = lane; b < nP; b += 64) inP[P[b]] = 1;
    } else {
        lh_reset(Wl, Wg, pmax);
    }
    WSYNC();
    bool warming = str != nullptr && !resume;
    bool w_valid = resume ? shared_int[1] != 0 : true;
    bool first_resumed = resume && nP > 0;
    if (stats && lane == 0) stats[7] += 1.0;
    for (int itn = 0; itn < 6 * n + 20; ++itn) {
        long long lt0 = stats ? wall_clock64() : 0;
        double best = wtol;
        int bidx = -1;
        bool do_append = true;
        if (first_resumed) {
            first_resumed = false, do_append = false;
        } else if (warming) {
            best = 100.0;
            for (int a = lane; a < n; a += 64)
                if (str[a] > best) best = str[a], bidx = a;
            wave_argmax(best, bidx);
            if (bidx >= 0 && lane == 0) str[bidx] = 0.0;
            WSYNC();
            if (bidx < 0 || nP >= pmax - 8) {
                warming = false, do_append = false;
                if (nP == 0) continue;
            }
        } else {
            double acc[4] = {0, 0, 0, 0};
            for (int q0 = 0; q0 < nP; q0 += 64) {
                const int pl = q0 + lane < nP ? P[q0 + lane] : -1;
                const double zl = pl >= 0 ? zc[pl] : 0.0;
                const int nb = nP - q0 < 64 ? nP - q0 : 64;
                for (int b0 = 0; b0 < nb; b0 += 4) {
                    double sv[4][4], zb[4];
#pragma unroll
                    for (int u = 0; u < 4; ++u) {
                        const int bb = b0 + u < nb ? b0 + u : nb - 1;
                        const int pb = __builtin_amdgcn_readlane(pl, bb);
                        zb[u] = b0 + u < nb ? rl_dyn(zl, bb) : 0.0;
                        const double* row = Sg + (size_t)pb * ldS;
#pragma unroll
                        for (int v = 0; v < 4; ++v) sv[u][v] = lane + 64 * v < n ? row[lane + 64 * v] : 0.0;
                    }
#pragma unroll
                    for (int u = 0; u < 4; ++u)
#pragma unroll
                        for (int v = 0; v < 4; ++v) acc[v] += sv[u][v] * zb[u];
                }
            }
#pragma unroll
            for (int v = 0; v < 4; ++v) {
                const int a = lane + 64 * v;
                if (a < n) {
                    const double s = dv[a] - acc[v];
                    if (!inP[a] && !banned[a] && s > best) best = s, bidx = a;
                }
            }
            wave_argmax(best, bidx);
            if (stats && lane == 0) { const long long t_ = wall_clock64(); stats[0] += (double)(t_ - lt0); lt0 = t_; stats[4] += 1.0; }
            if (bidx < 0) break;
        }
        const int j = bidx;
        if (do_append) {
            if (nP >= pmax) return -1;
            double sr[LH_H], lr[LH_H], wr[LH_H], tr[LH_H];
#pragma unroll
            for (int h = 0; h < LH_H; ++h) sr[h] = lane + 64 * h < nP ? Sg[(size_t)P[lane + 64 * h] * ldS + j] : 0.0;
            lh_rows(Wl, Wg, sr, lr, nP, lane);
            lhv_load(wv, wr, nP, lane);
            double ll = 0, lw = 0;
#pragma unroll
            for (int h = 0; h < LH_H; ++h) ll += lr[h] * lr[h], lw += w_valid ? lr[h] * wr[h] : 0.0;
            ll = wave_red(ll, 0);
            const double sjj = Sg[(size_t)j * ldS + j];
            const double djj = sjj - ll;
            if (!(djj > 1e-13 * fmax(1e-30, sjj))) {
                if (lane == 0) banned[j] = 1;
                WSYNC();
                continue;
            }
            lw = wave_red(lw, 0);
            lh_cols(Wl, Wg, lr, tr, nP, lane);
            const double ir = fast_rsqrt(djj);
            {
                const int rowo = lhp_row(nP), len = lhp_len(nP >> 3);
#pragma unroll
                for (int h = 0; h < LH_H; ++h) {
                    const int cq = lane + 64 * h;
                    if (cq < len) Lc[rowo + cq] = cq < nP ? -ir * tr[h] : (cq == nP ? ir : 0.0);
                }
            }
            if (lane == 0) {
                P[nP] = j;
                inP[j] = 1;
                wv[nP] = (dv[j] - lw) * ir;
            }
            nP++;
            WSYNC();
            if (stats && lane == 0) { const long long t_ = wall_clock64(); stats[1] += (double)(t_ - lt0); lt0 = t_; stats[5] += 1.0; }
        }
        if (warming) continue;
        for (int inner = 0; inner < 2 * pmax; ++inner) {
            {
                double wr[LH_H], yr[LH_H];
                if (!w_valid) {
                    double dr[LH_H];
#pragma unroll
                    for (int h = 0; h < LH_H; ++h) dr[h] = lane + 64 * h < nP ? dv[P[lane + 64 * h]] : 0.0;
                    lh_rows(Wl, Wg, dr, wr, nP, lane);
                    lhv_store(wv, wr, nP, lane);
                    w_valid = true;
                } else
                    lhv_load(wv, wr, nP, lane);
                lh_cols(Wl, Wg, wr, yr, nP, lane);
                lhv_store(yv, yr, nP, lane);
                WSYNC();
                if (stats && lane == 0) stats[6] += 1.0;
            }
            double ymin = 1e300;
            for (int b = lane; b < nP; b += 64) ymin = fmin(ymin, yv[b]);
            ymin = wave_red(ymin, 2);
            if (ymin > 0) {
                for (int b = lane; b < nP; b += 64) zc[P[b]] = yv[b];
                WSYNC();
                if (stats && lane == 0) { const long long t_ = wall_clock64(); stats[2] += (double)(t_ - lt0); lt0 = t_; }
                break;
            }
            double alpha = 1e300;
            for (int b = lane; b < nP; b += 64)
                if (yv[b] <= 0) alpha = fmin(alpha, zc[P[b]] / (zc[P[b]] - yv[b]));
            alpha = wave_red(alpha, 2);
            if (stats && lane == 0) { const long long t_ = wall_clock64(); stats[2] += (double)(t_ - lt0); lt0 = t_; }
            if (!(alpha >= 0)) alpha = 0;
            for (int b = lane; b < nP; b += 64) zc[P[b]] += alpha * (yv[b] - zc[P[b]]);
            WSYNC();
            if (lane == 0) {
                int nrem = 0, worst = 0;
                for (int b = 1; b < nP; ++b)
                    if (yv[b] < yv[worst]) worst = b;
                for (int b = 0; b < nP; ++b) {
                    const int ia = P[b];
                    if (yv[b] <= 0 && zc[ia] <= 1e-14 * fmax(1.0, fabs(yv[b]))) rem[nrem++] = b;
                }
                if (nrem == 0) rem[nrem++] = worst;
                *shared_int = nrem;
            }
            WSYNC();
            const int nrem = *shared_int;
            for (int q = nrem - 1; q >= 0; --q) {
                const int pos = rem[q];
                lh_delete(Wl, Wg, yv, nP, pos, lane);
                if (lane == 0) {
                    const int ia = P[pos];
                    zc[ia] = 0, inP[ia] = 0;
                    for (int b = pos; b < nP - 1; ++b) P[b] = P[b + 1];
                }
                nP--;
                WSYNC();
            }
            for (int a = lane; a < n; a += 64) banned[a] = 0;
            w_valid = false;
            WSYNC();
            if (stats && lane == 0) { const long long t_ = wall_clock64(); stats[3] += (double)(t_ - lt0); lt0 = t_; }
            if (nP == 0) break;
        }
    }
    if (lane == 0) shared_int[1] = w_valid ? 1 : 0;
    return nP;
}

__device__ __forceinline__ int polish_qp(RowCtx& c, PassIO& io, const PolishWs& pw, double* lds, double* red, int* flag, int mode) {
    const bool geometric = mode == 1, big = mode == 2;
    const QpDims& d = c.d;
    const QpWs& w = c.w;
    const int tid = threadIdx.x, NK = d.nk, nred = d.nj * NK;
    double* ctrl = const_cast<double*>(c.ctrl);
    const int pmax = big ? PL_PBIG : polish_pmax(NK);
    double* Lc = big ? pw.Lbig : lds;
    double* zc = big ? lds : lds + lhp_size(pmax);
    double* dv = zc + PL_NC;
    double* tv = dv + PL_NC;
    double* yv = tv + pmax;
    double* wv = yv + pmax;
    int* P = (int*)(wv + pmax);
    int* inP = P + pmax;
    int* banned = inP + PL_NC;
    int* sint = banned + PL_NC;
    double* str = (double*)(sint + 4);
    double* f3 = str + PL_NC;

#ifdef QP_LHSTATS
#define QP_PPROF_ON 0
#else
#define QP_PPROF_ON 1
#endif
#ifdef QP_PROFILE
    double* pscal = c.scal + 20;
    long long pt0 = wall_clock64();
#define PPROF(i)                                       \
    do {                                               \
        __syncthreads();                               \
        const long long t_ = wall_clock64();           \
        if (tid == 0 && QP_PPROF_ON) pscal[i] += (double)(t_ - pt0);  \
        pt0 = t_;                                      \
    } while (0)
#else
#define PPROF(i)
#endif
    if (tid == 0) pw.ncand[0] = 0;
    __threadfence_block();
    __syncthreads();
    if (geometric)
        row_pass<PASS_CAND_GEO>(c, io);
    else
        row_pass<PASS_CAND>(c, io);
    __threadfence_block();
    __syncthreads();
    if (pw.ncand[0] > PL_NC) return 1;

    k0_factor3(d, w, f3, flag);
    if (*flag) return 2;

    for (int it0 = tid; it0 < d.nb * 3 * d.oq; it0 += 4 * QP_THREADS) {
        double xq[4][6], sc4[4];
#pragma unroll
        for (int q = 0; q < 4; ++q) {
            const int it = it0 + q * QP_THREADS < d.nb * 3 * d.oq ? it0 + q * QP_THREADS : it0;
            const int a = it / (3 * d.oq), k = (it / d.oq) % 3, j6 = it % d.oq, m = j6 / 6;
            const double* xs = ctrl + ((size_t)(d.first + a) * 3 + k) * d.oq + 6 * m;
#pragma unroll
            for (int jj = 0; jj < 6; ++jj) xq[q][jj] = xs[jj];
            sc4[q] = w.segsc[m];
        }
#pragma unroll
        for (int q = 0; q < 4; ++q) {
            const int it = it0 + q * QP_THREADS;
            if (it < d.nb * 3 * d.oq) {
                const int i = (it % d.oq) % 6;
                double g = 0;
#pragma unroll
                for (int jj = 0; jj < 6; ++jj) g += Qbase[6 * i + jj] * xq[q][jj];
                w.cvec[it] = 2 * sc4[q] * g;
            }
        }
    }
    __threadfence_block();
    __syncthreads();
    apply_FT(d, w, w.cvec, pw.V, 1.0);
    __threadfence_block();
    __syncthreads();

    PPROF(0);
    bool accepted = false;
    int n_done = -1, nP = 0;
    for (int outer = 0; outer < 8 && !accepted; ++outer) {
        const int n = pw.ncand[0];
        if (n > PL_NC) return 1;
        const int n_prev = n_done < 0 ? 0 : n_done;
        const int first_new = n_done < 0 ? 0 : n_done;
        {
            const int n_new = n - first_new;
            for (int i = tid; i < n_new; i += QP_THREADS) inP[i] = pw.cand[first_new + i].row;
            __syncthreads();
            Cand mine;
            int rank = 0;
            if (tid < n_new) {
                mine = pw.cand[first_new + tid];
                for (int j = 0; j < n_new; ++j) rank += inP[j] < mine.row;
            }
            __syncthreads();
            if (tid < n_new) pw.cand[first_new + rank] = mine;
            __threadfence_block();
            __syncthreads();
        }
        for (int ci = tid; ci < n; ci += QP_THREADS) inP[ci] = cand_meta(pw.cand[ci]);
        __syncthreads();
        for (int it = tid; it < (n - first_new) * 6 * d.nj; it += QP_THREADS) {
            const int ci = first_new + it / (6 * d.nj), rem = it % (6 * d.nj), sk = rem / d.nj, jj = rem % d.nj, side = sk / 3, k = sk % 3;
            const int meta = inP[ci], ag = side == 0 ? (meta & 255) : ((meta >> 8) & 255) - 1;
            if (ag < 0 || !(((meta >> 16) >> k) & 1)) continue;
            double* v3 = pw.V + (size_t)(1 + ci) * nred + (size_t)jj * NK + (ag * 3 + k) * 3;
            v3[0] = 0.0, v3[1] = 0.0, v3[2] = 0.0;
        }
        __threadfence_block();
        __syncthreads();
        for (int it = tid; it < (n - first_new) * 18; it += QP_THREADS) {
            const int ci = first_new + it / 18, e18 = it % 18, side = e18 / 9, k = (e18 / 3) % 3, e = e18 % 3;
            const Cand& cd = pw.cand[ci];
            const int ag = side == 0 ? cd.a : cd.b;
            if (ag < 0 || cd.n[k] == 0.0) continue;
            const double sgn = side == 0 ? 1.0 : -1.0;
            pw.V[(size_t)(1 + ci) * nred + (size_t)(cd.knot - 1) * NK + (ag * 3 + k) * 3 + e] = sgn * cd.n[k] * cd.t[e];
        }
        __threadfence_block();
        __syncthreads();
        if (n_done < 0)
            col_solve3(d, pw, f3, true, 0, n);
        else if (n > n_done)
            col_solve3(d, pw, f3, false, n_done, n);
        n_done = n;
        __threadfence_block();
        __syncthreads();
        for (int it = tid; it < n * n; it += QP_THREADS) {
            const int ci = it / n, cj = it % n;
            if (cj > ci || ci < first_new) continue;
            const int ma = inP[ci], mb = inP[cj];
            const int aa = ma & 255, ab = ((ma >> 8) & 255) - 1, ba = mb & 255, bb = ((mb >> 8) & 255) - 1;
            bool share = aa == ba || (bb >= 0 && aa == bb) || (ab >= 0 && (ab == ba || ab == bb));
            if (share && ab < 0 && bb < 0) share = ((ma & mb) >> 16) != 0;
            double sv = 0.0;
            if (share) {
                const Cand& ca = pw.cand[ci];
                const Cand& cb = pw.cand[cj];
                sv = 0.5 * (cand_dot(ca, pw.V + (size_t)(1 + cj) * nred, NK, mb) + cand_dot(cb, pw.V + (size_t)(1 + ci) * nred, NK, ma));
            }
            pw.Sg[(size_t)ci * PL_NC + cj] = sv;
            pw.Sg[(size_t)cj * PL_NC + ci] = sv;
        }
        for (int ci = tid; ci < n; ci += QP_THREADS) dv[ci] = -cand_dot(pw.cand[ci], pw.V, NK) - pw.cand[ci].slack;
        for (int ci = tid; ci < n; ci += QP_THREADS)
            str[ci] = outer == 0 ? pw.cand[ci].strength : (ci < n_prev && zc[ci] > 0 ? 1e3 + zc[ci] : 0.0);
        __threadfence_block();
        __syncthreads();
        const double* Suse = pw.Sg;
        int ldS = PL_NC;
        {
            double* Sl = f3 + 18 * d.nj;
            if ((int)(Sl - lds) + n * n <= c.lds_avail) {
                for (int it = tid; it < n * n; it += QP_THREADS) Sl[it] = pw.Sg[(size_t)(it / n) * PL_NC + it % n];
                Suse = Sl, ldS = n;
                __syncthreads();
            }
        }
        PPROF(1);
        if (tid < 64) {
            __builtin_amdgcn_s_setprio(QP_CHAIN_PRIO);
            const int res_nP = (outer > 0 && nP > 0) ? nP : -1;
#ifdef QP_LHSTATS
            const int r = lh_wave(n, Suse, ldS, dv, zc, tv, yv, wv, P, inP, banned, Lc, sint + 2, pmax, str, big, c.scal + 20, res_nP, n_prev);
#else
            const int r = lh_wave(n, Suse, ldS, dv, zc, tv, yv, wv, P, inP, banned, Lc, sint + 2, pmax, str, big, nullptr, res_nP, n_prev);
#endif
            __builtin_amdgcn_s_setprio(0);
            if (tid == 0) sint[1] = r;
        }
        __syncthreads();
        nP = sint[1];
        PPROF(2);
        if (nP < 0) return 3;
        for (int round = 0; round < 4; ++round) {
            int* pcol = banned;
            int* pmeta = inP;
            for (int b = tid; b < nP; b += QP_THREADS) tv[b] = zc[P[b]], pcol[b] = 1 + P[b], pmeta[b] = cand_meta(pw.cand[P[b]]);
            __syncthreads();
            constexpr int POL_IPT = 3;
            for (int i0 = tid; i0 < nred; i0 += POL_IPT * QP_THREADS) {
                int ii[POL_IPT], ag[POL_IPT], kd[POL_IPT];
                double q[POL_IPT][8];
#pragma unroll
                for (int t = 0; t < POL_IPT; ++t) {
                    const int i = i0 + t * QP_THREADS;
                    ii[t] = i < nred ? i : -1;
                    const int sub = ((i < nred ? i : 0) % NK) / 3;
                    ag[t] = sub / 3, kd[t] = sub % 3;
#pragma unroll
                    for (int u = 0; u < 8; ++u) q[t][u] = 0.0;
                }
                int b = 0;
                for (; b + 8 <= nP; b += 8) {
                    double vv[POL_IPT][8];
#pragma unroll
                    for (int t = 0; t < POL_IPT; ++t)
#pragma unroll
                        for (int u = 0; u < 8; ++u)
                            vv[t][u] = (ii[t] >= 0 && meta_has(pmeta[b + u], ag[t], kd[t])) ? pw.V[(size_t)pcol[b + u] * nred + ii[t]] : 0.0;
#pragma unroll
                    for (int t = 0; t < POL_IPT; ++t)
#pragma unroll
                        for (int u = 0; u < 8; ++u) q[t][u] += tv[b + u] * vv[t][u];
                }
                for (; b < nP; ++b) {
                    double vv[POL_IPT];
#pragma unroll
                    for (int t = 0; t < POL_IPT; ++t) vv[t] = (ii[t] >= 0 && meta_has(pmeta[b], ag[t], kd[t])) ? pw.V[(size_t)pcol[b] * nred + ii[t]] : 0.0;
#pragma unroll
                    for (int t = 0; t < POL_IPT; ++t) q[t][0] += meta_has(pmeta[b], ag[t], kd[t]) ? tv[b] * vv[t] : 0.0;
                }
#pragma unroll
                for (int t = 0; t < POL_IPT; ++t)
                    if (ii[t] >= 0)
                        w.rhs[ii[t]] = -pw.V[ii[t]] - (((q[t][0] + q[t][1]) + (q[t][2] + q[t][3])) + ((q[t][4] + q[t][5]) + (q[t][6] + q[t][7])));
            }
            __threadfence_block();
            __syncthreads();
            apply_F(d, w, w.rhs, w.dx);
            __threadfence_block();
            __syncthreads();
            io.vmax = 0;
            row_pass<PASS_VERIFY>(c, io);
            const double vmax = block_reduce(io.vmax, 1, red);
            __threadfence_block();
            __syncthreads();
            if (pw.ncand[0] > n) break;
            double emax = 0, zmin = 0, zmax = 0;
            for (int b = tid; b < nP; b += QP_THREADS) {
                const double e = w.ds[pw.cand[P[b]].row];
                yv[b] = -e;
                emax = fmax(emax, fabs(e));
                zmin = fmin(zmin, zc[P[b]]), zmax = fmax(zmax, zc[P[b]]);
            }
            emax = block_reduce(emax, 1, red);
            zmin = block_reduce(zmin, 2, red);
            zmax = block_reduce(zmax, 1, red);
#ifdef QP_POLSTATS
            if (tid == 0) {
                double* ps = c.scal + 20;
                ps[0] = vmax, ps[1] = zmin, ps[2] = zmax, ps[3] = emax + 1000.0 * round + 1e6 * outer + 1e8 * nP + 1e12 * n;
            }
#endif
            if (vmax <= 5e-9 && zmin >= -1e-9 * fmax(1.0, zmax) && (emax < 1e-12 || round == 3)) {
                accepted = true;
                if (tid == 0) red[12] = fmax(fmax(vmax, 0.0), fmax(0.0, -zmin) / fmax(1.0, zmax));
                break;
            }
            if (round == 3) break;
            if (tid < 64 && nP > 0) {
                const int lane = tid;
                double er[LH_H], ur[LH_H], yr[LH_H];
                kl_lds* Wl = big ? nullptr : (kl_lds*)Lc;
                double* Wg = big ? Lc : nullptr;
                lhv_load(yv, er, nP, lane);
                lh_rows(Wl, Wg, er, ur, nP, lane);
                lh_cols(Wl, Wg, ur, yr, nP, lane);
#pragma unroll
                for (int h = 0; h < LH_H; ++h)
                    if (lane + 64 * h < nP) zc[P[lane + 64 * h]] += yr[h];
            }
            __syncthreads();
        }
        PPROF(3);
        if (!accepted && pw.ncand[0] <= n) break;
    }
    if (!accepted) return 4;
    {
        double* xb = ctrl + (size_t)d.first * 3 * d.oq;
        const int nx = d.nb * 3 * d.oq;
        for (int i0 = tid; i0 < nx; i0 += 4 * QP_THREADS) {
            double xv[4], dv4[4];
#pragma unroll
            for (int q = 0; q < 4; ++q) {
                const int i = i0 + q * QP_THREADS;
                xv[q] = i < nx ? xb[i] : 0.0, dv4[q] = i < nx ? w.dx[i] : 0.0;
            }
#pragma unroll
            for (int q = 0; q < 4; ++q)
                if (i0 + q * QP_THREADS < nx) xb[i0 + q * QP_THREADS] = xv[q] + dv4[q];
        }
    }
    __threadfence_block();
    __syncthreads();
    for (int b = tid; b < nP; b += QP_THREADS) {
        const Cand& cd = pw.cand[P[b]];
        if (cd.snap_idx >= 0 && zc[P[b]] > 0) ctrl[cd.snap_idx] = cd.snap_val;
    }
    __threadfence_block();
    __syncthreads();
    return 0;
}

template <class T>
__device__ __forceinline__ T uni_words(const T& v) {
    static_assert(sizeof(T) % 4 == 0, "whole words");
    union U {
        T t;
        unsigned wd[sizeof(T) / 4];
        __device__ U() {}
    } in, out;
    in.t = v;
#pragma unroll
    for (unsigned i = 0; i < sizeof(T) / 4; ++i) out.wd[i] = __builtin_amdgcn_readfirstlane(in.wd[i]);
    return out.t;
}
__device__ __noinline__ int polish_entry(RowCtx c_in, PolishWs pw_in, double* lds, double* red, int* flag, int mode) {
    PassIO io = {};
    RowCtx c = uni_words(c_in);
    PolishWs pw = uni_words(pw_in);
    c.pw = &pw;
    return polish_qp(c, io, pw, uni(lds), uni(red), uni(flag), uni(mode));
}
#endif
```

Measured before the change: 178,500.

## Precompute per-mission explicit K0 inverse table to replace per-candidate column solves in polish

Builds a per-mission table holding the explicit block inverse G of the K0 factor, computed with double-double arithmetic for accuracy and then symmetrised. The polish step then forms the candidate Schur matrix S by bilinear lookups into G, and forms the right-hand side via a sparse scatter table and a G product, instead of running triangular solves per candidate column and storing a large V array. This removes repeated per-candidate solves and the large V workspace. In exchange it adds a one-time table setup, which is O(nj^2) in storage and work, and the mission constants move into that setup step.

```diff
diff --git a/swarm_simulator_amd/csrc/common/ipm_rows.h b/swarm_simulator_amd/csrc/common/ipm_rows.h
--- a/swarm_simulator_amd/csrc/common/ipm_rows.h
+++ b/swarm_simulator_amd/csrc/common/ipm_rows.h
@@ -135,31 +135,75 @@
     return a_lo ? n0 * (d0 - f0) + n1 * (d1 - f1) + n2 * (d2 - f2) : n0 * (f0 - d0) + n1 * (f1 - d1) + n2 * (f2 - d2);
 }
 
-IPM_ROW bool k0_factor_step(double* f, double (&Bp)[9], bool first) {
+struct dd {
+    double h, l;
+    IPM_ROW dd() : h(0), l(0) {}
+    IPM_ROW dd(double x) : h(x), l(0) {}
+    IPM_ROW dd(double hh, double ll) : h(hh), l(ll) {}
+};
+IPM_ROW dd dd_quick(double a, double b) {
+    const double s = a + b;
+    return dd(s, b - (s - a));
+}
+IPM_ROW dd dd_sum(double a, double b) {
+    const double s = a + b, bb = s - a;
+    return dd(s, (a - (s - bb)) + (b - bb));
+}
+IPM_ROW dd operator+(dd a, dd b) {
+    dd s = dd_sum(a.h, b.h);
+    const dd t = dd_sum(a.l, b.l);
+    s = dd_quick(s.h, s.l + t.h);
+    return dd_quick(s.h, s.l + t.l);
+}
+IPM_ROW dd operator-(dd a) { return dd(-a.h, -a.l); }
+IPM_ROW dd operator-(dd a, dd b) { return a + (-b); }
+IPM_ROW dd operator*(dd a, dd b) {
+    const double p = a.h * b.h;
+    return dd_quick(p, fma(a.h, b.h, -p) + (a.h * b.l + a.l * b.h));
+}
+IPM_ROW dd operator/(dd a, dd b) {
+    const double q1 = a.h / b.h;
+    dd r = a - b * dd(q1);
+    const double q2 = r.h / b.h;
+    r = r - b * dd(q2);
+    const double q3 = r.h / b.h;
+    return dd_quick(q1, q2) + dd(q3);
+}
+IPM_ROW dd& operator-=(dd& a, dd b) { return a = a - b; }
+IPM_ROW bool operator>(dd a, dd b) { return a.h > b.h || (a.h == b.h && a.l > b.l); }
+IPM_ROW double k0_sqrt(double a) { return sqrt(a); }
+IPM_ROW dd k0_sqrt(dd a) {
+    const double x = 1.0 / sqrt(a.h), ax = a.h * x;
+    return dd_sum(ax, (a - dd(ax) * dd(ax)).h * (x * 0.5));
+}
+
+template <class T>
+IPM_ROW bool k0_factor_step(T* f, T (&Bp)[9], bool first) {
     bool ok = true;
-    double A[9], Ej[9];
+    T A[9], Ej[9];
     for (int e = 0; e < 9; ++e) A[e] = f[e], Ej[e] = f[9 + e];
     if (!first)
         for (int r = 0; r < 3; ++r)
             for (int c = 0; c < 3; ++c) A[3 * r + c] -= Bp[3 * r] * Bp[3 * c] + Bp[3 * r + 1] * Bp[3 * c + 1] + Bp[3 * r + 2] * Bp[3 * c + 2];
-    if (!(A[0] > 0)) ok = false;
-    const double l00 = sqrt(A[0]), l10 = A[3] / l00, l20 = A[6] / l00;
-    const double d11 = A[4] - l10 * l10;
-    if (!(d11 > 0)) ok = false;
-    const double l11 = sqrt(d11), l21 = (A[7] - l20 * l10) / l11;
-    const double d22 = A[8] - l20 * l20 - l21 * l21;
-    if (!(d22 > 0)) ok = false;
-    const double l22 = sqrt(d22);
-    f[0] = 1.0 / l00, f[1] = 0, f[2] = 0, f[3] = l10, f[4] = 1.0 / l11, f[5] = 0, f[6] = l20, f[7] = l21, f[8] = 1.0 / l22;
+    const T zero = T(0.0), one = T(1.0);
+    if (!(A[0] > zero)) ok = false;
+    const T l00 = k0_sqrt(A[0]), l10 = A[3] / l00, l20 = A[6] / l00;
+    const T d11 = A[4] - l10 * l10;
+    if (!(d11 > zero)) ok = false;
+    const T l11 = k0_sqrt(d11), l21 = (A[7] - l20 * l10) / l11;
+    const T d22 = A[8] - l20 * l20 - l21 * l21;
+    if (!(d22 > zero)) ok = false;
+    const T l22 = k0_sqrt(d22);
+    f[0] = one / l00, f[1] = zero, f[2] = zero, f[3] = l10, f[4] = one / l11, f[5] = zero, f[6] = l20, f[7] = l21, f[8] = one / l22;
     for (int r = 0; r < 3; ++r) {
-        const double o0 = Ej[r], o1 = Ej[3 + r], o2 = Ej[6 + r];
-        const double x0 = o0 / l00, x1 = (o1 - x0 * l10) / l11, x2 = (o2 - x0 * l20 - x1 * l21) / l22;
+        const T o0 = Ej[r], o1 = Ej[3 + r], o2 = Ej[6 + r];
+        const T x0 = o0 / l00, x1 = (o1 - x0 * l10) / l11, x2 = (o2 - x0 * l20 - x1 * l21) / l22;
         f[9 + 3 * r] = Bp[3 * r] = x0, f[10 + 3 * r] = Bp[3 * r + 1] = x1, f[11 + 3 * r] = Bp[3 * r + 2] = x2;
     }
     return ok;
 }
-template <class F>
-IPM_ROW void k0_forward_step(F f, bool link, double (&y)[3], const double (&p)[3]) {
+template <class F, class T>
+IPM_ROW void k0_forward_step(F f, bool link, T (&y)[3], const T (&p)[3]) {
     if (link) {
         const F Bm = f - 9;
         y[0] -= Bm[0] * p[0] + Bm[1] * p[1] + Bm[2] * p[2];
@@ -170,8 +214,8 @@
     y[1] = (y[1] - f[3] * y[0]) * f[4];
     y[2] = (y[2] - f[6] * y[0] - f[7] * y[1]) * f[8];
 }
-template <class F>
-IPM_ROW void k0_backward_step(F f, bool link, double (&y)[3], const double (&p)[3]) {
+template <class F, class T>
+IPM_ROW void k0_backward_step(F f, bool link, T (&y)[3], const T (&p)[3]) {
     if (link) {
         const F Bm = f + 9;
         y[0] -= Bm[0] * p[0] + Bm[3] * p[1] + Bm[6] * p[2];
@@ -183,4 +227,59 @@
     y[0] = (y[0] - f[3] * y[1] - f[6] * y[2]) * f[0];
 }
 
-}
+IPM_ROW size_t k0g_block(int ja, int jb) { return 9 * ((size_t)ja * (ja + 1) / 2 + jb); }
+IPM_ROW size_t k0g_doubles(int nj) { return k0g_block(nj, 0); }
+template <class P>
+IPM_ROW double k0g_at(P G, int ja, int r, int jb, int c) {
+    return ja >= jb ? G[k0g_block(ja, jb) + 3 * r + c] : G[k0g_block(jb, ja) + 3 * c + r];
+}
+template <class P>
+IPM_ROW double k0g_bilinear(P blk, bool a_first, const double (&ta)[3], const double (&tb)[3]) {
+    const double (&tr)[3] = a_first ? ta : tb;
+    const double (&tc)[3] = a_first ? tb : ta;
+    return tr[0] * (blk[0] * tc[0] + blk[1] * tc[1] + blk[2] * tc[2]) + tr[1] * (blk[3] * tc[0] + blk[4] * tc[1] + blk[5] * tc[2]) +
+           tr[2] * (blk[6] * tc[0] + blk[7] * tc[1] + blk[8] * tc[2]);
+}
+constexpr int K0_BLK = 6;
+template <class F, class P>
+IPM_ROW void k0_inverse_column(F f, int nj, int jb, int c, P G, P lo) {
+    dd p[3];
+    for (int ja = jb; ja < nj; ++ja) {
+        dd y[3];
+        if (ja == jb) y[0] = dd(c == 0 ? 1.0 : 0.0), y[1] = dd(c == 1 ? 1.0 : 0.0), y[2] = dd(c == 2 ? 1.0 : 0.0);
+        k0_forward_step(f + 18 * ja, ja > jb, y, p);
+        const size_t o = k0g_block(ja, jb) + c;
+        for (int e = 0; e < 3; ++e) p[e] = y[e], G[o + 3 * e] = y[e].h, lo[o + 3 * e] = y[e].l;
+    }
+    constexpr int B = K0_BLK;
+    dd cur[B][3], nxt[B][3];
+    for (int u = 0; u < B; ++u) {
+        const int jx = nj - 1 - u >= jb ? nj - 1 - u : jb;
+        const size_t o = k0g_block(jx, jb) + c;
+        for (int e = 0; e < 3; ++e) cur[u][e] = dd(G[o + 3 * e], lo[o + 3 * e]);
+    }
+    for (int jt = nj - 1; jt >= jb; jt -= B) {
+        for (int u = 0; u < B; ++u) {
+            const int jx = jt - B - u >= jb ? jt - B - u : jb;
+            const size_t o = k0g_block(jx, jb) + c;
+            for (int e = 0; e < 3; ++e) nxt[u][e] = dd(G[o + 3 * e], lo[o + 3 * e]);
+        }
+        for (int u = 0; u < B; ++u) {
+            const int jj = jt - u;
+            if (jj >= jb) {
+                k0_backward_step(f + 18 * jj, jj + 1 < nj, cur[u], p);
+                const size_t o = k0g_block(jj, jb) + c;
+                for (int e = 0; e < 3; ++e) p[e] = cur[u][e], G[o + 3 * e] = cur[u][e].h;
+            }
+        }
+        for (int u = 0; u < B; ++u)
+            for (int e = 0; e < 3; ++e) cur[u][e] = nxt[u][e];
+    }
+}
+template <class P>
+IPM_ROW void k0g_symmetrise(P blk) {
+    const double a = 0.5 * (blk[1] + blk[3]), b = 0.5 * (blk[2] + blk[6]), c = 0.5 * (blk[5] + blk[7]);
+    blk[1] = blk[3] = a, blk[2] = blk[6] = b, blk[5] = blk[7] = c;
+}
+
+}
diff --git a/swarm_simulator_amd/csrc/kernels/qp.hip b/swarm_simulator_amd/csrc/kernels/qp.hip
--- a/swarm_simulator_amd/csrc/kernels/qp.hip
+++ b/swarm_simulator_amd/csrc/kernels/qp.hip
@@ -75,8 +75,9 @@
 #define PL_PMAX 160
 #define PL_PBIG 192
 __host__ __device__ inline int polish_pmax(int nk) { return nk <= 36 ? 112 : PL_PMAX; }
+__host__ __device__ inline size_t polish_s_doubles(int nj) { return std::max((size_t)PL_NC * PL_NC, ipm::k0g_doubles(nj)); }
 __host__ __device__ inline size_t polish_ws_doubles(int nj, int nk) {
-    return PL_NC * 14 + (size_t)(PL_NC + 1) * nj * nk + PL_NC * PL_NC + 8 + lhp_size(PL_PBIG);
+    return 18 * (size_t)nj + 2 + ipm::k0g_doubles(nj) + PL_NC * 14 + polish_s_doubles(nj) + 8 + lhp_size(PL_PBIG) + 4 * 6 * PL_PBIG + 3 * (size_t)nj * nk;
 }
 __host__ __device__ inline int polish_lds_doubles(int nk) {
     const int pm = polish_pmax(nk);
@@ -2197,7 +2198,6 @@
     const QpDims& d = c.d;
     const QpWs& w = c.w;
     const int M = d.M;
-    mission_constants(d, T, const_cast<QpWs&>(w));
     init_block_pads(d, w);
 
     {
@@ -2473,12 +2473,7 @@
     const double blk_doubles = d.nk <= 36 ? 5.0 * (d.nk * (d.nk + 1) / 2) + 5.0 * d.nk : 8.0 * d.ldb * d.ldb;
     const double bytes_sweeps = 88.0 * frozen_free_rows + 64.0 * (double)(d.oq - 6) * (6.0 * d.nb + 2.0 * d.npb) + 288.0 * (double)d.nb * (d.oq - 6);
     const double bytes_iter = bytes_sweeps + 8.0 * (double)d.nj * blk_doubles;
-    PolishWs pw;
-    pw.cand = (Cand*)w.polish;
-    pw.V = w.polish + PL_NC * 14;
-    pw.Sg = pw.V + (size_t)(PL_NC + 1) * d.nj * d.nk;
-    pw.ncand = (int*)(pw.Sg + PL_NC * PL_NC);
-    pw.Lbig = pw.Sg + PL_NC * PL_NC + 8;
+    const PolishWs pw = polish_carve(w.polish, d.nj);
     row_pass<PASS_INIT>(c, io);
     __threadfence_block();
     __syncthreads();
@@ -2734,6 +2729,22 @@
     }
 }
 
+__device__ __noinline__ void mission_tables(const DevSession* Sg, double* ws_base, size_t ws_stride, int mission, int nbmax) {
+    const DevSession& S = *Sg;
+    ws_base = uni(ws_base), mission = uni(mission), nbmax = uni(nbmax);
+    if (S.status[mission] != 0) return;
+    const int N = S.N, M = __builtin_amdgcn_readfirstlane(S.Mk[mission]);
+    const QpDims d = make_dims(N, M, 0, min(nbmax, N));
+    QpWs w = carve(ws_base + (size_t)mission * ws_stride, d, nbmax);
+    mission_constants(d, S.T + (size_t)mission * (S.M + 1), w);
+    __threadfence_block();
+    __syncthreads();
+    extern __shared__ __attribute__((aligned(16))) double lds_raw[];
+    k0_mission_tables(d.nj, w, polish_carve(w.polish, d.nj), lds_raw + 32);
+    __threadfence_block();
+    __syncthreads();
+}
+
 __device__ __noinline__ int qp_batch_body_outofline(const DevSession* Sg, double* ws_base, size_t ws_stride, int mission, int batch, int nbmax,
                                                     int reset_cost, int lds_doubles, int pass_index, double far_R) {
     const DevSession S = *Sg;
@@ -2772,6 +2783,7 @@
     __shared__ DevSession S_lds;
     if (threadIdx.x == 0) S_lds = S;
     __syncthreads();
+    mission_tables(&S_lds, ws_base, ws_stride, mission, nbmax);
     int stop_it = -1, stop_l = 0;
     for (int it = 0; it < passes && stop_it < 0; ++it)
         for (int l = 0; l < biter; ++l) {
@@ -2821,6 +2833,7 @@
     const int nkw = std::min(nk, 36);
     size_t lds = sizeof(double) * (2 * (size_t)((nk + 15) & ~15) + QP_THREADS + 32) + 16;
     lds = std::max(lds, sizeof(double) * (size_t)(std::max(polish_lds_doubles(nk), polish_lds_doubles(nkw)) + 18 * (M - 1) + 32) + 16);
+    lds = std::max(lds, sizeof(double) * (size_t)(54 * (M - 1) + 32) + 16);
     lds = std::max(lds, sizeof(double) * (16 + (size_t)QP_STAGE_BUFS * 2 * (nkw * KL_LD + KL_I) + (size_t)(M - 1) * nkw + 2 + 6 * KS_VLEN + 2 * 64 + 64));
     lds = std::max(lds, sizeof(double) * (size_t)(2 * kl_area_doubles(nkw) + 128 + (QP_FOLLOW_ASM ? 2 : ASM_HELPERS) * ASML_DOUBLES(nkw, nkw / 9) + 32) + 16);
     if (nk > 36 && nk <= 72) {
diff --git a/swarm_simulator_amd/csrc/kernels/qp_polish.inc b/swarm_simulator_amd/csrc/kernels/qp_polish.inc
--- a/swarm_simulator_amd/csrc/kernels/qp_polish.inc
+++ b/swarm_simulator_amd/csrc/kernels/qp_polish.inc
@@ -10,11 +10,26 @@
 
 struct PolishWs {
     Cand* cand;
-    double* V;
+    double* v0;
     double* Sg;
     int* ncand;
     double* Lbig;
+    double* ptab;
+    double* k0f;
+    double* G;
 };
+__device__ __forceinline__ PolishWs polish_carve(double* p, int nj) {
+    PolishWs pw;
+    pw.k0f = p, p += 18 * (size_t)nj + 2;
+    pw.G = p, p += k0g_doubles(nj);
+    pw.cand = (Cand*)p, p += PL_NC * 14;
+    pw.Sg = p, p += polish_s_doubles(nj);
+    pw.ncand = (int*)p, p += 8;
+    pw.Lbig = p, p += lhp_size(PL_PBIG);
+    pw.ptab = p, p += 4 * 6 * PL_PBIG;
+    pw.v0 = p;
+    return pw;
+}
 
 #define WSYNC()                                             \
     do {                                                    \
@@ -64,21 +79,19 @@
 __device__ __forceinline__ int cand_meta(const Cand& c) {
     return c.a | ((c.b + 1) << 8) | ((c.n[0] != 0.0) << 16) | ((c.n[1] != 0.0) << 17) | ((c.n[2] != 0.0) << 18);
 }
-__device__ __forceinline__ bool meta_has(int meta, int agent, int k) {
-    return meta < 0 || ((((meta >> 16) >> k) & 1) && (agent == (meta & 255) || agent == ((meta >> 8) & 255) - 1));
-}
-__device__ __forceinline__ double cand_dot(const Cand& c, const double* vec, int nk, int colmeta = -1) {
+__device__ __forceinline__ int meta_sign(int meta, int agent, int k) {
+    if (!(((meta >> 16) >> k) & 1)) return 0;
+    return agent == (meta & 255) ? 1 : (agent == ((meta >> 8) & 255) - 1 ? -1 : 0);
+}
+__device__ __forceinline__ double cand_dot(const Cand& c, const double* vec, int nk) {
     const double* blk = vec + (size_t)(c.knot - 1) * nk;
     double s = 0;
 #pragma unroll
     for (int k = 0; k < 3; ++k) {
         if (c.n[k] == 0.0) continue;
-        double ta = 0;
-        if (meta_has(colmeta, c.a, k)) {
-            const double* pa = blk + (c.a * 3 + k) * 3;
-            ta = c.t[0] * pa[0] + c.t[1] * pa[1] + c.t[2] * pa[2];
-        }
-        if (c.b >= 0 && meta_has(colmeta, c.b, k)) {
+        const double* pa = blk + (c.a * 3 + k) * 3;
+        double ta = c.t[0] * pa[0] + c.t[1] * pa[1] + c.t[2] * pa[2];
+        if (c.b >= 0) {
             const double* pb = blk + (c.b * 3 + k) * 3;
             ta -= c.t[0] * pb[0] + c.t[1] * pb[1] + c.t[2] * pb[2];
         }
@@ -87,23 +100,37 @@
     return s;
 }
 
-__device__ void k0_factor3(const QpDims& d, const QpWs& w, double* f3, int* flag) {
-    for (int it = threadIdx.x; it < 18 * d.nj; it += QP_THREADS) {
+__device__ void k0_mission_tables(int nj, const QpWs& w, const PolishWs& pw, double* lds) {
+    double* f3 = lds;
+    dd* fd = (dd*)(lds + 18 * nj);
+    for (int it = threadIdx.x; it < 18 * nj; it += QP_THREADS) {
         const int jj = it / 18, e = it % 18, j = jj + 1;
-        f3[it] = e < 9 ? w.Dk[9 * j + e] : (jj + 1 < d.nj ? w.Ek[9 * j + (e - 9)] : 0.0);
+        const double v = e < 9 ? w.Dk[9 * j + e] : (jj + 1 < nj ? w.Ek[9 * j + (e - 9)] : 0.0);
+        f3[it] = v, fd[it] = dd(v);
     }
     __syncthreads();
     if (threadIdx.x == 0) {
         int ok = 1;
         double Bp[9] = {0, 0, 0, 0, 0, 0, 0, 0, 0};
-        for (int jj = 0; jj < d.nj; ++jj)
+        for (int jj = 0; jj < nj; ++jj)
             if (!k0_factor_step(f3 + 18 * jj, Bp, jj == 0)) ok = 0;
-        *flag = !ok;
-    }
-    __syncthreads();
-}
-
-constexpr int K0_BLK = 6;
+        *(int*)(pw.k0f + 18 * (size_t)nj) = !ok;
+    }
+    if (threadIdx.x == 64) {
+        int ok = 1;
+        dd Bd[9];
+        for (int jj = 0; jj < nj; ++jj)
+            if (!k0_factor_step(fd + 18 * jj, Bd, jj == 0)) ok = 0;
+        *((int*)(pw.k0f + 18 * (size_t)nj) + 1) = !ok;
+    }
+    __syncthreads();
+    for (int it = threadIdx.x; it < 18 * nj; it += QP_THREADS) pw.k0f[it] = f3[it];
+    for (int col = threadIdx.x; col < 3 * nj; col += QP_THREADS) k0_inverse_column((const dd*)fd, nj, col / 3, col % 3, pw.G, pw.Sg);
+    __threadfence_block();
+    __syncthreads();
+    for (int jj = threadIdx.x; jj < nj; jj += QP_THREADS) k0g_symmetrise(pw.G + k0g_block(jj, jj));
+}
+
 __device__ __forceinline__ void k0_solve3(const double* f3g, int nj, int nk, double* col, int sub) {
     typedef __attribute__((address_space(1))) double gdb;
     const kl_lds* f3 = (const kl_lds*)f3g;
@@ -165,29 +192,65 @@
     }
 }
 
-__device__ __noinline__ void col_solve3_fn(int nj_v, int nk_v, int nb_v, double* V_v, const Cand* cand_v, const double* f3_v, int with_grad_v, int c0_v, int c1_v) {
+__device__ __noinline__ void v0_solve3_fn(int nj_v, int nk_v, int nb_v, double* v0_v, const double* f3_v) {
     const int nj = __builtin_amdgcn_readfirstlane(nj_v), nk = __builtin_amdgcn_readfirstlane(nk_v), nb = __builtin_amdgcn_readfirstlane(nb_v);
-    const int with_grad = __builtin_amdgcn_readfirstlane(with_grad_v), c0 = __builtin_amdgcn_readfirstlane(c0_v), c1 = __builtin_amdgcn_readfirstlane(c1_v);
-    double* V = uni(V_v);
-    const Cand* cand = uni(cand_v);
+    double* v0 = uni(v0_v);
     const double* f3 = uni(f3_v);
-    const int nred = nj * nk, ng = with_grad ? nb * 3 : 0;
-    for (int it = threadIdx.x; it < ng + (c1 - c0) * 6; it += QP_THREADS) {
-        if (it < ng) {
-            k0_solve3(f3, nj, nk, V, it);
-            continue;
-        }
-        const int ci = c0 + (it - ng) / 6, side = ((it - ng) % 6) / 3, k = (it - ng) % 3;
-        const Cand& cd = cand[ci];
-        const int ag = side == 0 ? cd.a : cd.b;
-        if (ag < 0 || cd.n[k] == 0.0) continue;
-        k0_solve3(f3, nj, nk, V + (size_t)(1 + ci) * nred, ag * 3 + k);
-    }
-}
-__device__ __forceinline__ void col_solve3(const QpDims& d, const PolishWs& pw, const double* f3, bool with_grad, int c0, int c1) {
-    col_solve3_fn(d.nj, d.nk, d.nb, pw.V, pw.cand, f3, with_grad ? 1 : 0, c0, c1);
-    __threadfence_block();
-    __syncthreads();
+    for (int it = threadIdx.x; it < nb * 3; it += QP_THREADS) k0_solve3(f3, nj, nk, v0, it);
+}
+
+__device__ __noinline__ void table_product_fn(int nj_v, int nk_v, int nb_v, const double* G_v, const double* u_v, double* out_v) {
+    typedef __attribute__((address_space(1))) const double gcd;
+    const int nj = __builtin_amdgcn_readfirstlane(nj_v), nk = __builtin_amdgcn_readfirstlane(nk_v), nsub = 3 * __builtin_amdgcn_readfirstlane(nb_v);
+    gcd* G = QGC(uni(G_v));
+    gcd* uv = QGC(uni(u_v));
+    double* out = uni(out_v);
+    constexpr int PB = 4;
+    for (int it = threadIdx.x; it < nj * nsub; it += QP_THREADS) {
+        const int jj = it / nsub, sub = it % nsub;
+        double acc[3] = {0, 0, 0};
+        for (int k0 = 0; k0 < nj; k0 += PB) {
+            double g[PB][9], x[PB][3];
+#pragma unroll
+            for (int u = 0; u < PB; ++u) {
+                const int kb = k0 + u < nj ? k0 + u : nj - 1;
+                gcd* blk = G + (jj >= kb ? k0g_block(jj, kb) : k0g_block(kb, jj));
+#pragma unroll
+                for (int e = 0; e < 9; ++e) g[u][e] = blk[e];
+#pragma unroll
+                for (int e = 0; e < 3; ++e) x[u][e] = uv[(size_t)kb * nk + sub * 3 + e];
+            }
+#pragma unroll
+            for (int u = 0; u < PB; ++u) {
+                if (k0 + u >= nj) continue;
+                if (jj >= k0 + u) {
+                    acc[0] += g[u][0] * x[u][0] + g[u][1] * x[u][1] + g[u][2] * x[u][2];
+                    acc[1] += g[u][3] * x[u][0] + g[u][4] * x[u][1] + g[u][5] * x[u][2];
+                    acc[2] += g[u][6] * x[u][0] + g[u][7] * x[u][1] + g[u][8] * x[u][2];
+                } else {
+                    acc[0] += g[u][0] * x[u][0] + g[u][3] * x[u][1] + g[u][6] * x[u][2];
+                    acc[1] += g[u][1] * x[u][0] + g[u][4] * x[u][1] + g[u][7] * x[u][2];
+                    acc[2] += g[u][2] * x[u][0] + g[u][5] * x[u][1] + g[u][8] * x[u][2];
+                }
+            }
+        }
+        const size_t i = (size_t)jj * nk + sub * 3;
+#pragma unroll
+        for (int e = 0; e < 3; ++e) out[i + e] = -acc[e];
+    }
+}
+
+__device__ __forceinline__ double s_from_table(const Cand* cand, const double* G, int ci, int cj, int ma, int mb) {
+    const int aa = ma & 255, ab = ((ma >> 8) & 255) - 1, ba = mb & 255, bb = ((mb >> 8) & 255) - 1;
+    const int sg = (aa == ba) - (bb >= 0 && aa == bb) - (ab >= 0 && ab == ba) + (ab >= 0 && ab == bb);
+    bool share = aa == ba || (bb >= 0 && aa == bb) || (ab >= 0 && (ab == ba || ab == bb));
+    if (share && ab < 0 && bb < 0) share = ((ma & mb) >> 16) != 0;
+    if (!share || sg == 0) return 0.0;
+    const Cand& ca = cand[ci];
+    const Cand& cb = cand[cj];
+    const bool a_first = ca.knot >= cb.knot;
+    const double* blk = G + k0g_block((a_first ? ca.knot : cb.knot) - 1, (a_first ? cb.knot : ca.knot) - 1);
+    return (double)sg * (ca.n[0] * cb.n[0] + ca.n[1] * cb.n[1] + ca.n[2] * cb.n[2]) * k0g_bilinear(blk, a_first, ca.t, cb.t);
 }
 
 __device__ __forceinline__ double rl_dyn(double v, int lane) {
@@ -396,7 +459,7 @@
     const bool geometric = mode == 1, big = mode == 2;
     const QpDims& d = c.d;
     const QpWs& w = c.w;
-    const int tid = threadIdx.x, NK = d.nk, nred = d.nj * NK;
+    const int tid = threadIdx.x, NK = d.nk;
     double* ctrl = const_cast<double*>(c.ctrl);
     const int pmax = big ? PL_PBIG : polish_pmax(NK);
     double* Lc = big ? pw.Lbig : lds;
@@ -441,8 +504,11 @@
     __syncthreads();
     if (pw.ncand[0] > PL_NC) return 1;
 
-    k0_factor3(d, w, f3, flag);
-    if (*flag) return 2;
+    {
+        const int* k0bad = (const int*)(pw.k0f + 18 * (size_t)d.nj);
+        if (k0bad[0] | k0bad[1]) return 2;
+    }
+    for (int it = tid; it < 18 * d.nj; it += QP_THREADS) f3[it] = pw.k0f[it];
 
     for (int it0 = tid; it0 < d.nb * 3 * d.oq; it0 += 4 * QP_THREADS) {
         double xq[4][6], sc4[4];
@@ -469,18 +535,29 @@
     }
     __threadfence_block();
     __syncthreads();
-    apply_FT(d, w, w.cvec, pw.V, 1.0);
+    double* gred = pw.v0 + (size_t)d.nj * NK;
+    double* usum = gred + (size_t)d.nj * NK;
+    apply_FT(d, w, w.cvec, gred, 1.0);
+    __threadfence_block();
+    __syncthreads();
+    for (int i = tid; i < d.nj * NK; i += QP_THREADS) pw.v0[i] = gred[i];
+    __threadfence_block();
+    __syncthreads();
+    v0_solve3_fn(d.nj, d.nk, d.nb, pw.v0, f3);
     __threadfence_block();
     __syncthreads();
 
     PPROF(0);
     bool accepted = false;
-    int n_done = -1, nP = 0;
+    int n_done = 0, nP = 0;
     for (int outer = 0; outer < 8 && !accepted; ++outer) {
         const int n = pw.ncand[0];
         if (n > PL_NC) return 1;
-        const int n_prev = n_done < 0 ? 0 : n_done;
-        const int first_new = n_done < 0 ? 0 : n_done;
+        const int n_prev = n_done;
+#ifndef QP_PROFILE
+        if (outer > 0 && tid == 0) c.scal[SC_PROF0 + 4] += 1;
+#endif
+        const int first_new = n_done;
         {
             const int n_new = n - first_new;
             for (int i = tid; i < n_new; i += QP_THREADS) inP[i] = pw.cand[first_new + i].row;
@@ -497,50 +574,16 @@
             __syncthreads();
         }
         for (int ci = tid; ci < n; ci += QP_THREADS) inP[ci] = cand_meta(pw.cand[ci]);
-        __syncthreads();
-        for (int it = tid; it < (n - first_new) * 6 * d.nj; it += QP_THREADS) {
-            const int ci = first_new + it / (6 * d.nj), rem = it % (6 * d.nj), sk = rem / d.nj, jj = rem % d.nj, side = sk / 3, k = sk % 3;
-            const int meta = inP[ci], ag = side == 0 ? (meta & 255) : ((meta >> 8) & 255) - 1;
-            if (ag < 0 || !(((meta >> 16) >> k) & 1)) continue;
-            double* v3 = pw.V + (size_t)(1 + ci) * nred + (size_t)jj * NK + (ag * 3 + k) * 3;
-            v3[0] = 0.0, v3[1] = 0.0, v3[2] = 0.0;
-        }
-        __threadfence_block();
-        __syncthreads();
-        for (int it = tid; it < (n - first_new) * 18; it += QP_THREADS) {
-            const int ci = first_new + it / 18, e18 = it % 18, side = e18 / 9, k = (e18 / 3) % 3, e = e18 % 3;
-            const Cand& cd = pw.cand[ci];
-            const int ag = side == 0 ? cd.a : cd.b;
-            if (ag < 0 || cd.n[k] == 0.0) continue;
-            const double sgn = side == 0 ? 1.0 : -1.0;
-            pw.V[(size_t)(1 + ci) * nred + (size_t)(cd.knot - 1) * NK + (ag * 3 + k) * 3 + e] = sgn * cd.n[k] * cd.t[e];
-        }
-        __threadfence_block();
-        __syncthreads();
-        if (n_done < 0)
-            col_solve3(d, pw, f3, true, 0, n);
-        else if (n > n_done)
-            col_solve3(d, pw, f3, false, n_done, n);
         n_done = n;
-        __threadfence_block();
         __syncthreads();
         for (int it = tid; it < n * n; it += QP_THREADS) {
             const int ci = it / n, cj = it % n;
             if (cj > ci || ci < first_new) continue;
-            const int ma = inP[ci], mb = inP[cj];
-            const int aa = ma & 255, ab = ((ma >> 8) & 255) - 1, ba = mb & 255, bb = ((mb >> 8) & 255) - 1;
-            bool share = aa == ba || (bb >= 0 && aa == bb) || (ab >= 0 && (ab == ba || ab == bb));
-            if (share && ab < 0 && bb < 0) share = ((ma & mb) >> 16) != 0;
-            double sv = 0.0;
-            if (share) {
-                const Cand& ca = pw.cand[ci];
-                const Cand& cb = pw.cand[cj];
-                sv = 0.5 * (cand_dot(ca, pw.V + (size_t)(1 + cj) * nred, NK, mb) + cand_dot(cb, pw.V + (size_t)(1 + ci) * nred, NK, ma));
-            }
+            const double sv = s_from_table(pw.cand, pw.G, ci, cj, inP[ci], inP[cj]);
             pw.Sg[(size_t)ci * PL_NC + cj] = sv;
             pw.Sg[(size_t)cj * PL_NC + ci] = sv;
         }
-        for (int ci = tid; ci < n; ci += QP_THREADS) dv[ci] = -cand_dot(pw.cand[ci], pw.V, NK) - pw.cand[ci].slack;
+        for (int ci = tid; ci < n; ci += QP_THREADS) dv[ci] = -cand_dot(pw.cand[ci], pw.v0, NK) - pw.cand[ci].slack;
         for (int ci = tid; ci < n; ci += QP_THREADS)
             str[ci] = outer == 0 ? pw.cand[ci].strength : (ci < n_prev && zc[ci] > 0 ? 1e3 + zc[ci] : 0.0);
         __threadfence_block();
@@ -571,49 +614,56 @@
         nP = sint[1];
         PPROF(2);
         if (nP < 0) return 3;
+        int* pmeta = inP;
+        int* off = banned;
+        const int nsub = 3 * d.nb;
+        for (int b = tid; b < nP; b += QP_THREADS) pmeta[b] = cand_meta(pw.cand[P[b]]);
+        __syncthreads();
+        for (int sub = tid; sub < nsub; sub += QP_THREADS) {
+            int cnt = 0;
+            for (int b = 0; b < nP; ++b) cnt += meta_sign(pmeta[b], sub / 3, sub % 3) != 0;
+            ((int*)str)[sub] = cnt;
+        }
+        __syncthreads();
+        for (int sub = tid; sub <= nsub; sub += QP_THREADS) {
+            int o = 0;
+            for (int q = 0; q < sub; ++q) o += ((int*)str)[q];
+            off[sub] = o;
+        }
+        __syncthreads();
+        for (int it = tid; it < nP * 6; it += QP_THREADS) {
+            const int b = it / 6, side = (it % 6) / 3, k = it % 3;
+            const int meta = pmeta[b], ag = side == 0 ? (meta & 255) : ((meta >> 8) & 255) - 1;
+            if (ag < 0 || !(((meta >> 16) >> k) & 1)) continue;
+            int rank = 0;
+            for (int q = 0; q < b; ++q) rank += meta_sign(pmeta[q], ag, k) != 0;
+            const Cand& cd = pw.cand[P[b]];
+            const double sn = side == 0 ? cd.n[k] : -cd.n[k];
+            double* en = pw.ptab + 4 * (size_t)(off[ag * 3 + k] + rank);
+            en[0] = (double)((cd.knot - 1) * 1024 + b), en[1] = sn * cd.t[0], en[2] = sn * cd.t[1], en[3] = sn * cd.t[2];
+        }
+        __threadfence_block();
+        __syncthreads();
         for (int round = 0; round < 4; ++round) {
-            int* pcol = banned;
-            int* pmeta = inP;
-            for (int b = tid; b < nP; b += QP_THREADS) tv[b] = zc[P[b]], pcol[b] = 1 + P[b], pmeta[b] = cand_meta(pw.cand[P[b]]);
-            __syncthreads();
-            constexpr int POL_IPT = 3;
-            for (int i0 = tid; i0 < nred; i0 += POL_IPT * QP_THREADS) {
-                int ii[POL_IPT], ag[POL_IPT], kd[POL_IPT];
-                double q[POL_IPT][8];
-#pragma unroll
-                for (int t = 0; t < POL_IPT; ++t) {
-                    const int i = i0 + t * QP_THREADS;
-                    ii[t] = i < nred ? i : -1;
-                    const int sub = ((i < nred ? i : 0) % NK) / 3;
-                    ag[t] = sub / 3, kd[t] = sub % 3;
-#pragma unroll
-                    for (int u = 0; u < 8; ++u) q[t][u] = 0.0;
+            for (int b = tid; b < nP; b += QP_THREADS) tv[b] = zc[P[b]];
+            __syncthreads();
+            for (int it = tid; it < d.nj * nsub; it += QP_THREADS) {
+                const int kb = it / nsub, sub = it % nsub;
+                const size_t i = (size_t)kb * NK + sub * 3;
+                double u0 = gred[i], u1 = gred[i + 1], u2 = gred[i + 2];
+                for (int o = off[sub]; o < off[sub + 1]; ++o) {
+                    const double* en = pw.ptab + 4 * (size_t)o;
+                    const int key = (int)en[0];
+                    if ((key >> 10) == kb) {
+                        const double zb = tv[key & 1023];
+                        u0 += zb * en[1], u1 += zb * en[2], u2 += zb * en[3];
+                    }
                 }
-                int b = 0;
-                for (; b + 8 <= nP; b += 8) {
-                    double vv[POL_IPT][8];
-#pragma unroll
-                    for (int t = 0; t < POL_IPT; ++t)
-#pragma unroll
-                        for (int u = 0; u < 8; ++u)
-                            vv[t][u] = (ii[t] >= 0 && meta_has(pmeta[b + u], ag[t], kd[t])) ? pw.V[(size_t)pcol[b + u] * nred + ii[t]] : 0.0;
-#pragma unroll
-                    for (int t = 0; t < POL_IPT; ++t)
-#pragma unroll
-                        for (int u = 0; u < 8; ++u) q[t][u] += tv[b + u] * vv[t][u];
-                }
-                for (; b < nP; ++b) {
-                    double vv[POL_IPT];
-#pragma unroll
-                    for (int t = 0; t < POL_IPT; ++t) vv[t] = (ii[t] >= 0 && meta_has(pmeta[b], ag[t], kd[t])) ? pw.V[(size_t)pcol[b] * nred + ii[t]] : 0.0;
-#pragma unroll
-                    for (int t = 0; t < POL_IPT; ++t) q[t][0] += meta_has(pmeta[b], ag[t], kd[t]) ? tv[b] * vv[t] : 0.0;
-                }
-#pragma unroll
-                for (int t = 0; t < POL_IPT; ++t)
-                    if (ii[t] >= 0)
-                        w.rhs[ii[t]] = -pw.V[ii[t]] - (((q[t][0] + q[t][1]) + (q[t][2] + q[t][3])) + ((q[t][4] + q[t][5]) + (q[t][6] + q[t][7])));
-            }
+                usum[i] = u0, usum[i + 1] = u1, usum[i + 2] = u2;
+            }
+            __threadfence_block();
+            __syncthreads();
+            table_product_fn(d.nj, NK, d.nb, pw.G, usum, w.rhs);
             __threadfence_block();
             __syncthreads();
             apply_F(d, w, w.rhs, w.dx);
```

Result: faster. 188,300 (median of 6 runs) (+5.5%).
